# albtad01/NBody-EuroHPC

Measured on AMD Instinct MI355X. Metric: body-interactions/s, higher is better.
Workload: dtype f32; 1 GPU; murb galaxy N=200000 steps=451 dt=3600 soft=2e8 seed=0 fp32 — BASELINE.json configs[2]: N=200000 i=200, 1 x MI355X; n_bodies=200000, parallelism=1 gpu, kernel_variant=8, jsplit=1, sym_waves=4, taper_pct=5, sym_passes=1

## Files before the change

### nbody-eurohpc_amd/csrc/murb_choose.h

```cpp
#ifndef MURB_CHOOSE_H_
#define MURB_CHOOSE_H_

#include <algorithm>
#include <cstddef>

#include "murb_layout.h"
#include "murb_plan.h"

namespace {

struct PlanInputs {
    unsigned long n = 0;
    int world = 1;
    unsigned long slice = 0;
    unsigned long slots = 0;
    int cu_count = 0;
    size_t device_mem = 0;
    int resident_per_cu = 0;
    int variant = 0, jsplit = 0;
    int sym_waves = 0;
    int taper = -1;
    int diag_tri = -1;
    int sym_red = -1;
    int fuse_integrate = 1;
    long sym_pass_mb = 0;
    int tri_div = 0;
};

constexpr int kMaxParts = 64;
constexpr int kNumVariants = 8;
constexpr int kOneSidedVariant = 1;
constexpr int kOneSidedFewBodies = 2;
constexpr int kPersistentVariant = 7;
constexpr int kSymmetricVariant = 8;
constexpr unsigned long kSymmetricMinBodies = 2049;
constexpr int kRowsPerLaunch = kMaxParts / 2;

struct Plan {
    int variant;
    int parts_local, parts_remote;
    bool persistent;
    bool symmetric;
    int split;
    int waves;
    int taper;
    bool diag_tri;
    int red;
    MurbSchedule sched[2];
};

constexpr double kSymFastMaxReach = 0x1p34;
constexpr double kSymFastMinSoft = 0x1p-40;
inline bool sym_wide_needed(double reach, double soft) { return !(reach <= kSymFastMaxReach && soft >= kSymFastMinSoft); }
inline bool sym_wide_chosen(int option, bool needed) { return option < 0 ? needed : option != 0; }

inline int resident_blocks(const PlanInputs& in) { return std::max(in.resident_per_cu, 1) * std::max(in.cu_count, 1); }

inline MurbSchedule make_schedule(const PlanInputs& in, long groups, long tiles, int row_base)
{
    MurbSchedule sc{(int)groups, (int)tiles, 1, row_base};
    const long units = groups * tiles;
    if (units <= 0) { sc.nblocks = 0; return sc; }
    const long slots = resident_blocks(in);
    long rounds = in.jsplit > 0 ? in.jsplit : std::min<long>(8, std::max<long>(1, units / (slots * 8)));
    long nb = std::min(units, slots * rounds);
    nb = std::min(nb, std::max<long>(1, (kRowsPerLaunch - 2) * groups));
    sc.nblocks = (int)std::max<long>(nb, 1);
    return sc;
}

inline int variant_group(int variant)
{
    switch (variant) {
        case kPersistentVariant: return 32;
        case kSymmetricVariant: return 32;
        case 2: case 6: return 16;
        case 5: return 64;
        default: return 32;
    }
}

inline int auto_parts(const PlanInputs& in, int variant, unsigned long i_slots, unsigned long tiles)
{
    if (tiles == 0) return 0;
    const unsigned long groups = (i_slots + variant_group(variant) - 1) / variant_group(variant);
    const unsigned long want_blocks = (unsigned long)std::max(in.cu_count, 1) * 6ul * 24ul;
    unsigned long parts = (want_blocks + groups - 1) / groups;
    parts = std::min(parts, std::max(tiles / 8ul, 1ul));
    parts = std::max(parts, 1ul);
    return (int)std::min<unsigned long>(parts, kMaxParts / 2);
}

inline long sym_items_per_rank(const PlanInputs& in)
{
    const long tb = (long)(in.slice / MURB_SYM_BLOCK), w = in.world;
    return tb * (tb + 1) / 2 + ((w - 1) / 2) * tb * tb + (w > 1 && w % 2 == 0 ? tb * ((tb + 1) / 2) : 0);
}

inline size_t sym_pass_budget(const PlanInputs& in)
{
    if (in.sym_pass_mb > 0) return (size_t)in.sym_pass_mb << 20;
    return in.device_mem ? in.device_mem / 4 : 0;
}

inline size_t sym_row_bytes(const PlanInputs& in, int split)
{
    const size_t tb = in.slice / MURB_SYM_BLOCK, w = (size_t)in.world, far = w / 2;
    size_t rows = tb * tb + (size_t)(split - 1) * tb * (tb - 1) / 2;
    if (w > 1) rows += tb * far * tb + far * tb * (size_t)split * tb;
    return rows * MURB_SYM_BLOCK * 3 * sizeof(float);
}

inline bool fused_one_sided_wins(const PlanInputs& in)
{
    const unsigned long T = in.slots / MURB_SYM_BLOCK;
    return in.fuse_integrate && in.jsplit == 0 && (T <= 4 || T == 6);
}

inline Plan make_plan(const PlanInputs& in)
{
    Plan p{};
    const auto fits = [&](int split) { return in.world == 1 || in.device_mem == 0 || sym_row_bytes(in, split) < in.device_mem / 2; };
    if (in.variant >= 1 && in.variant <= kNumVariants) p.variant = in.variant;
    else if (in.world == 1) p.variant = (in.n >= kSymmetricMinBodies && !fused_one_sided_wins(in) && fits(1)) ? kSymmetricVariant : kOneSidedVariant;
    else p.variant = (sym_items_per_rank(in) >= 400 && fits(1)) ? kSymmetricVariant : (in.slice <= 16384 ? kOneSidedFewBodies : kOneSidedVariant);
    p.symmetric = p.variant == kSymmetricVariant;
    if (p.symmetric) {
        const long items = sym_items_per_rank(in);
        const long want = (in.world > 1 ? 16L : 8L) * 4 * std::max(in.cu_count, 1);
        p.split = (in.jsplit == 1 || in.jsplit == 2 || in.jsplit == 4 || in.jsplit == 8 || in.jsplit == 16)
                      ? in.jsplit
                      : (items >= want ? 1 : (2 * items >= want ? 2 : (in.world == 1 || items >= 1000 ? 4 : (items >= 400 ? 8 : 16))));
        struct SmallPlan { int waves, split, taper; bool diag_tri; };
        static const SmallPlan kSmallPlans[5] = {{8, 4, 30, true}, {4, 4, 5, false}, {4, 8, 5, false}, {8, 8, 30, true}, {4, 16, 5, false}};
        static const signed char kSmallPlanOfBlocks[25] = {4, 4, 4, 3, 3, 3, 4,
                                                           3, 3, 0, 2, 2, 1, 3, 0, 2, 1, 2, 0, 1, 2, 0, 1, 0, 2};
        const int T = (int)(in.slots / MURB_SYM_BLOCK);
        const bool small = in.world == 1 && T <= 27;
        const SmallPlan sp = kSmallPlans[(small && in.cu_count == 256 && T >= 3) ? kSmallPlanOfBlocks[T - 3] : (T < 10 ? 3 : 0)];
        p.waves = (in.sym_waves == 4 || in.sym_waves == 8) ? in.sym_waves : (small ? sp.waves : 4);
        if (in.jsplit == 0 && in.sym_waves == 0 && small) p.split = sp.split;
        while (p.split > 1 && MURB_SYM_BLOCK / p.split < 16 * p.waves) p.split /= 2;
        while (p.split > 1 && !fits(p.split)) p.split /= 2;
        p.taper = in.taper >= 0 ? in.taper : (in.world > 1 ? 0 : (small ? sp.taper : (in.n <= 600000 ? 5 : 0)));
        p.diag_tri = in.diag_tri >= 0 ? in.diag_tri != 0 : (small && sp.diag_tri);
        p.red = in.sym_red >= 0 ? in.sym_red : 1;
        p.persistent = false;
        p.parts_local = p.parts_remote = 0;
        return p;
    }
    const unsigned long tiles_local = in.slice / MURB_TILE_BODIES;
    const unsigned long tiles_remote = (in.slots - in.slice) / MURB_TILE_BODIES;
    p.persistent = p.variant == kPersistentVariant;
    if (p.persistent) {
        unsigned long first, count;
        partition(in.n, in.world, 0, &first, &count);
        const long groups = (long)((count + 31) / 32);
        p.sched[0] = make_schedule(in, groups, (long)tiles_local, 0);
        p.sched[1] = make_schedule(in, groups, (long)tiles_remote, kRowsPerLaunch);
        p.parts_local = p.parts_remote = 0;
        return p;
    }
    if (in.world == 1) {
        p.parts_local = in.jsplit > 0 ? std::min<int>(in.jsplit, (int)std::min<unsigned long>(tiles_local, kMaxParts))
                                      : auto_parts(in, p.variant, in.slice, tiles_local);
        if (in.jsplit == 0 && in.fuse_integrate && p.variant == kOneSidedVariant && in.slots / MURB_SYM_BLOCK <= 6) p.parts_local = 1;
        p.parts_remote = 0;
    } else {
        const unsigned long tiles_all = tiles_local + tiles_remote;
        int total = in.jsplit > 0 ? in.jsplit : auto_parts(in, p.variant, in.slice, tiles_all);
        total = std::max(total, 2);
        int loc = (int)std::max<unsigned long>(1ul, (unsigned long)total * tiles_local / tiles_all);
        int rem = std::max(1, total - loc);
        p.parts_local = (int)std::min<unsigned long>((unsigned long)loc, std::min<unsigned long>(tiles_local, kMaxParts / 2));
        p.parts_remote = (int)std::min<unsigned long>((unsigned long)rem, std::min<unsigned long>(tiles_remote, kMaxParts / 2));
    }
    return p;
}

inline int plan_tri_div(const PlanInputs& in, const Plan& p)
{
    if (in.tri_div > 0) return in.tri_div;
    if (in.world == 1) return 1;
    const long tb = (long)(in.slice / MURB_SYM_BLOCK);
    const long items = tb * (tb + 1) / 2 * p.split / 2;
    const long slots = 4L * std::max(in.cu_count, 1) * 4 / p.waves;
    int div = 1;
    while (div < 4 && items * div < 2 * slots && MURB_SYM_BLOCK / (p.split * div * 2) >= 16 * p.waves) div *= 2;
    return div;
}

inline SymLayoutKey sym_layout_key(const PlanInputs& in, const Plan& p, bool exchange_mode, int overlap, int tri_first_pct, bool xcd_order,
                                   bool pad_aware)
{
    SymLayoutKey k;
    k.split = p.split; k.waves = p.waves; k.taper = p.taper; k.diag_tri = p.diag_tri;
    k.exchange_mode = exchange_mode;
    k.overlap = exchange_mode ? overlap : 0;
    k.tri_first_pct = exchange_mode ? tri_first_pct : 0;
    k.xcd_order = xcd_order;
    k.budget_floats = sym_pass_budget(in) / (3 * sizeof(float));
    k.tri_div = plan_tri_div(in, p);
    k.pad_aware = pad_aware;
    return k;
}

inline int hermite_parts(const PlanInputs& in)
{
    const unsigned long tiles = in.slots / MURB_TILE_BODIES;
    if (in.jsplit > 0) return (int)std::min<unsigned long>((unsigned long)in.jsplit, std::min<unsigned long>(tiles, kMaxParts / 2));
    return auto_parts(in, kOneSidedFewBodies, in.slots, tiles);
}

}

#endif
```

### nbody-eurohpc_amd/csrc/murb_ctx.h

```cpp
#ifndef MURB_CTX_H_
#define MURB_CTX_H_

#include <hip/hip_runtime.h>

#include <vector>

#include "murb_choose.h"
#include "murb_crew.h"
#include "murb_kernels_block.h"
#include "murb_kernels_field.h"
#include "murb_kernels_sym.h"
#include "murb_kernels_tidal.h"
#include "murb_kernels_tracer.h"
#include "murb_kernels_knn.h"
#include "murb_rccl.h"

namespace {

inline int hip_rc(hipError_t e) { return e == hipSuccess ? 0 : -(int)e; }
inline int nccl_rc(int r) { return r == 0 ? 0 : -(3000 + r); }

template <typename... P> inline void release(P*... p) { ((void)hipFree((void*)p), ...); }
inline void release_event(hipEvent_t& e) { if (e) (void)hipEventDestroy(e); e = nullptr; }
inline void release_stream(hipStream_t& s) { if (s) (void)hipStreamDestroy(s); s = nullptr; }
inline void drain(hipStream_t s) { if (s) (void)hipStreamSynchronize(s); }

#define HIP_TRY(expr)                        \
    do {                                     \
        const int rc_ = hip_rc((expr));      \
        if (rc_ != 0) return rc_;            \
    } while (0)
#define RC_TRY(expr)                \
    do {                            \
        const int rc_ = (expr);     \
        if (rc_ != 0) return rc_;   \
    } while (0)

struct SymSet {
    float* part = nullptr;
    size_t comp_stride = 0;
    MurbSymBlockRows* rows = nullptr;
    int nblocks = 0;
    std::vector<SymPass> passes;
};

struct Shard {
    int device = 0;
    int rank = 0;
    unsigned long first = 0, count = 0;
    hipStream_t compute = nullptr, comm = nullptr;
    hipStream_t compute_low = nullptr;
    hipEvent_t ev_integrated = nullptr, ev_gathered = nullptr, ev_tri = nullptr;
    float4* rec[2] = {nullptr, nullptr};
    float4* vel = nullptr;
    float4* accp = nullptr;
    float* acc_out = nullptr;
    float* phi_out = nullptr;
    float* mass = nullptr;
    float* radius = nullptr;
    double* metrics = nullptr;
    double* metrics_host = nullptr;
    MurbSymItem* sym_items = nullptr;
    int sym_items_own = 0, sym_items_total = 0;
    SymLayoutKey key;
    int sym_red = 0;
    int sym_t1 = 0;
    SymSet sym_main;
    SymSet sym_tri;
    float* sym_send = nullptr;
    float* sym_recv = nullptr;
    float* sym_p2p = nullptr;
    float* sym_tri_acc = nullptr;
    double* sym_acc64 = nullptr;
    hipEvent_t ev_rowsum = nullptr, ev_reduced = nullptr;
    rccl_comm_t comm_rccl = nullptr;
    std::vector<hipEvent_t> prof;
    size_t prof_used = 0;
    std::vector<int> prof_kind;
    float4* herm_rec = nullptr;
    float4* herm_vel = nullptr;
    float* herm_a0 = nullptr;
    float* herm_j0 = nullptr;
    float4* herm_part = nullptr;
    int herm_rows = 0;
    MurbEvolveCtl* herm_ctl = nullptr;
    MurbEvolveCtl* herm_ctl_host = nullptr;
    MurbBlockCtl* blk_ctl = nullptr;
    MurbBlockCtl* blk_ctl_host = nullptr;
    unsigned int* blk_ticks = nullptr;
    int* blk_levels = nullptr;
    int* blk_list = nullptr;
    float4* blk_rec = nullptr;
    float4* blk_vel = nullptr;
    float4* blk_part = nullptr;
    size_t blk_rows = 0;
    int* nn_idx = nullptr;
    float* nn_r2 = nullptr;
    MurbEncList* enc = nullptr;
    float* herm_phi = nullptr;
    double* pot_sums = nullptr;
    double* pot_sums_host = nullptr;
    float* fld_in = nullptr;
    float4* fld_pts = nullptr;
    float* fld_out = nullptr;
    size_t fld_points = 0;
    float4* fld_part = nullptr;
    size_t fld_rows = 0;
    float* trc_state = nullptr;
    float4* trc_pts = nullptr;
    size_t trc_cap = 0;
    float4* trc_part = nullptr;
    size_t trc_rows = 0;
    float* knn_part_r2 = nullptr;
    int* knn_part_idx = nullptr;
    size_t knn_part = 0;
    float* knn_list_r2 = nullptr;
    int* knn_list_idx = nullptr;
    size_t knn_list = 0;
    float* knn_rho = nullptr;
    size_t knn_rhos = 0;
    double* knn_sums = nullptr;
    size_t knn_blocks = 0;
    unsigned long sym_launches = 0;
    size_t bytes = 0;
};

template <typename T>
int shard_alloc(Shard& sh, T*& p, size_t bytes, hipStream_t zero_on = nullptr)
{
    if (p) return 0;
    HIP_TRY(hipMalloc((void**)&p, bytes));
    sh.bytes += bytes;
    if (zero_on) HIP_TRY(hipMemsetAsync(p, 0, bytes, zero_on));
    return 0;
}
template <typename T>
void shard_free(Shard& sh, T*& p, size_t bytes)
{
    if (!p) return;
    release(p);
    p = nullptr;
    sh.bytes -= bytes;
}

constexpr int kPeSumBlocks = 256;
constexpr size_t kProfPairs = 4096;

enum ProfKind {
    kProfForce = 0,
    kProfTri1,
    kProfRect,
    kProfTri2,
    kProfReduceScatter,
    kProfAllGather,
    kProfWaitGather,
    kProfWaitReduce,
    kProfStep,
    kProfField,
    kProfTidal,
    kProfTracer,
    kProfKnn,
    kProfKinds
};

}

struct murbhip_ctx {
    PlanInputs in;
    float soft2 = 0.f, g = 0.f;
    int exchange = 0;
    bool rank_mode = false;
    std::vector<Shard> shards;
    ShardCrew* crew = nullptr;
    int cur = 0;
    bool uploaded = false;
    bool gather_pending = false;
    bool reduce_pending = false;
    int profile = 0, overlap = 1;
    int tri_first_pct = 50;
    int xcd_order = 0;
    int evolve_batch = 0;
    int integrator = 0;
    bool herm_current = false;
    bool herm_in_acc_out = false;
    bool herm_proposal = false;
    unsigned long evolve_steps = 0;
    int block_units = 0;
    bool blk_open = false;
    int blk_have_levels = 0;
    float blk_dt_max = 0.f;
    int blk_kmax = 0;
    double blk_steps_per_block = 0;
    double blk_info[4] = {0, 0, 0, 0};
    int nearest = 0;
    float enc_radius = 0.f;
    unsigned long enc_count = 0;
    double enc_time = 0.0;
    int contact = 0;
    int potential = 0;
    long field_chunks = 0;
    long field_batch = 0;
    unsigned long tracers = 0;
    bool trc_current = false;
    long tracer_chunks = 0;
    long tracer_batch = 0;
    int tracer_dt = 0;
    bool lf_half = false;
    bool acc_current = false;
    unsigned long state_serial = 1;
    unsigned long metrics_serial = 0;
    bool metrics_with_phi = false;
    double metrics_sums[MURB_METRIC_VALUES] = {0};
    bool want_pe = false;
    bool pe_current = false;
    float lf_last_dt = 0.f;
    int force_exchange = 0;
    int init_libm_fma = -1;
    int sym_wide = -1;
    bool sym_wide_needed = false;
    int energy_sweep = 0;
    int exchange_p2p = 0;
    int pad_aware = 1;
    int cu_reserve = 0;
    int solo_shard = -1;
    int clock_mhz = 0;
    double interactions_per_launch = 0;
    int async_error = 0;
};

#endif
```

### nbody-eurohpc_amd/csrc/murb_kernels_sym.h

```cpp
#ifndef MURB_KERNELS_SYM_H_
#define MURB_KERNELS_SYM_H_

#include "murb_kernels.h"
#include "murb_sym_types.h"

#ifndef MURB_SYM_STEP_BARRIER
#define MURB_SYM_STEP_BARRIER 1
#endif

struct MurbSymArgs {
    const float4* rec;
    float* part;
    unsigned long comp_stride;
    const MurbSymItem* items;
    int item_first;
    float soft2;
};

__device__ __forceinline__ void murb_swap32(float& a, float& b)
{
    asm volatile("s_nop 1\n\tv_permlane32_swap_b32 %0, %1\n\ts_nop 1" : "+v"(a), "+v"(b));
}
__device__ __forceinline__ void murb_swap16(float& a, float& b)
{
    asm volatile("s_nop 1\n\tv_permlane16_swap_b32 %0, %1\n\ts_nop 1" : "+v"(a), "+v"(b));
}
template <int CTRL> __device__ __forceinline__ float murb_dpp(float v)
{
    return __builtin_bit_cast(float, __builtin_amdgcn_update_dpp(0, __builtin_bit_cast(int, v), CTRL, 0xF, 0xF, true));
}

__device__ __forceinline__ float murb_reduce12(float (&v)[12], int lane)
{
    float w[6];
#pragma unroll
    for (int k = 0; k < 6; ++k) { murb_swap32(v[2 * k], v[2 * k + 1]); w[k] = v[2 * k] + v[2 * k + 1]; }
    float x[3];
#pragma unroll
    for (int m = 0; m < 3; ++m) { murb_swap16(w[2 * m], w[2 * m + 1]); x[m] = w[2 * m] + w[2 * m + 1]; }
    const bool b3 = (lane & 8) != 0, b2 = (lane & 4) != 0;
    const float keep3 = b3 ? x[1] : x[0], send3 = b3 ? x[0] : x[1];
    const float y0 = keep3 + murb_dpp<0x140>(send3);
    const float y1 = x[2] + murb_dpp<0x140>(x[2]);
    const float keep2 = b2 ? y1 : y0, send2 = b2 ? y0 : y1;
    float z = keep2 + murb_dpp<0x141>(send2);
    z += murb_dpp<0x4E>(z);
    z += murb_dpp<0xB1>(z);
    return z;
}

__device__ __forceinline__ float murb_masked(float v, unsigned mask)
{
    float out;
    asm("s_and_b32 %0, %1, %2" : "=s"(out) : "s"(v), "s"(mask) : "scc");
    return out;
}
__device__ __forceinline__ unsigned murb_ones_if_ge(int p, int threshold)
{
    unsigned out;
    asm("s_sub_i32 %0, %1, %2\n\ts_ashr_i32 %0, %0, 31" : "=s"(out) : "s"(threshold), "s"(p + 1) : "scc");
    return out;
}

template <int WIDE = 0>
__device__ __forceinline__ void murb_interact_sym(const murb_f2 xj, const murb_f2 yj, const murb_f2 zj, const murb_f2 gj,
                                                  const float xi, const float yi, const float zi, const float gi,
                                                  const float soft2, murb_f2& aix, murb_f2& aiy, murb_f2& aiz,
                                                  murb_f2& ajx, murb_f2& ajy, murb_f2& ajz)
{
    const murb_f2 dx = xj - xi;
    const murb_f2 dy = yj - yi;
    const murb_f2 dz = zj - zi;
    murb_f2 r2 = __builtin_elementwise_fma(dx, dx, (murb_f2)(soft2));
    r2 = __builtin_elementwise_fma(dy, dy, r2);
    r2 = __builtin_elementwise_fma(dz, dz, r2);
    murb_f2 inv;
    inv.x = __builtin_amdgcn_rsqf(r2.x);
    inv.y = __builtin_amdgcn_rsqf(r2.y);
    murb_f2 fi, fj;
    if constexpr (WIDE) {
        const murb_f2 inv2 = inv * inv;
        fi = (gj * inv) * inv2;
        fj = ((murb_f2)(-gi) * inv) * inv2;
    } else {
        const murb_f2 inv3 = (inv * inv) * inv;
        fi = gj * inv3;
        fj = inv3 * (-gi);
    }
    aix = __builtin_elementwise_fma(fi, dx, aix);
    aiy = __builtin_elementwise_fma(fi, dy, aiy);
    aiz = __builtin_elementwise_fma(fi, dz, aiz);
    ajx = __builtin_elementwise_fma(fj, dx, ajx);
    ajy = __builtin_elementwise_fma(fj, dy, ajy);
    ajz = __builtin_elementwise_fma(fj, dz, ajz);
}

template <int WIDE = 0>
__device__ __forceinline__ void murb_interact_sym_pe(const murb_f2 xj, const murb_f2 yj, const murb_f2 zj, const murb_f2 gj,
                                                     const float xi, const float yi, const float zi, const float gi, const float gi_pe,
                                                     const float soft2, murb_f2& aix, murb_f2& aiy, murb_f2& aiz,
                                                     murb_f2& ajx, murb_f2& ajy, murb_f2& ajz, murb_f2& pe)
{
    const murb_f2 dx = xj - xi;
    const murb_f2 dy = yj - yi;
    const murb_f2 dz = zj - zi;
    murb_f2 r2 = __builtin_elementwise_fma(dx, dx, (murb_f2)(soft2));
    r2 = __builtin_elementwise_fma(dy, dy, r2);
    r2 = __builtin_elementwise_fma(dz, dz, r2);
    murb_f2 inv;
    inv.x = __builtin_amdgcn_rsqf(r2.x);
    inv.y = __builtin_amdgcn_rsqf(r2.y);
    murb_f2 fi, fj, gg;
    if constexpr (WIDE) {
        const murb_f2 inv2 = inv * inv;
        gg = gj * inv;
        fi = gg * inv2;
        fj = ((murb_f2)(-gi) * inv) * inv2;
    } else {
        const murb_f2 inv3 = (inv * inv) * inv;
        fi = gj * inv3;
        fj = inv3 * (-gi);
        gg = gj * inv;
    }
    pe = __builtin_elementwise_fma(gg, (murb_f2)(gi_pe), pe);
    aix = __builtin_elementwise_fma(fi, dx, aix);
    aiy = __builtin_elementwise_fma(fi, dy, aiy);
    aiz = __builtin_elementwise_fma(fi, dz, aiz);
    ajx = __builtin_elementwise_fma(fj, dx, ajx);
    ajy = __builtin_elementwise_fma(fj, dy, ajy);
    ajz = __builtin_elementwise_fma(fj, dz, ajz);
}

__device__ __forceinline__ void murb_interact_sym_phi(const murb_f2 xj, const murb_f2 yj, const murb_f2 zj, const murb_f2 gj,
                                                      const float xi, const float yi, const float zi, const float gi,
                                                      const float soft2, murb_f2& phi_i, murb_f2& phi_j)
{
    const murb_f2 dx = xj - xi;
    const murb_f2 dy = yj - yi;
    const murb_f2 dz = zj - zi;
    murb_f2 r2 = __builtin_elementwise_fma(dx, dx, (murb_f2)(soft2));
    r2 = __builtin_elementwise_fma(dy, dy, r2);
    r2 = __builtin_elementwise_fma(dz, dz, r2);
    murb_f2 inv;
    inv.x = __builtin_amdgcn_rsqf(r2.x);
    inv.y = __builtin_amdgcn_rsqf(r2.y);
    phi_i = __builtin_elementwise_fma(gj, inv, phi_i);
    phi_j = __builtin_elementwise_fma(inv, (murb_f2)(gi), phi_j);
}

template <int WAVES, int ILOAD, int PHI, int RED, int DYN, int WIDE>
__device__ __forceinline__ void murb_sym_walk(const MurbSymArgs& a, const float4* tileA, const float4* tileB, float* stage,
                                              const int lane, const int wave, const int groups_per_wave,
                                              const unsigned int i_block_slot, const unsigned long out_off, const int out_stride,
                                              const float pe_scale, const int p_first,
                                              const int p_sym, murb_f2 (&ajx)[MURB_SYM_STEPS], murb_f2 (&ajy)[MURB_SYM_STEPS],
                                              murb_f2 (&ajz)[MURB_SYM_STEPS])
{
    constexpr int R = MURB_SYM_R;
    constexpr int NV = PHI == 2 ? 13 : 12;
    const float soft2 = a.soft2;
    const int stage_wr = lane;
    const int stage_rd = ((lane >> 2) < NV ? (lane >> 2) : NV - 1) * 80 + (lane & 3) * 4;
    const auto team_sum = [&](int g_of) {
        const float4* src = reinterpret_cast<const float4*>(stage + stage_rd);
        const float4 t0 = src[0], t1 = src[4], t2 = src[8], t3 = src[12];
        murb_f2 s2 = (murb_f2){t0.x, t0.y} + (murb_f2){t0.z, t0.w};
        s2 += (murb_f2){t1.x, t1.y}; s2 += (murb_f2){t1.z, t1.w};
        s2 += (murb_f2){t2.x, t2.y}; s2 += (murb_f2){t2.z, t2.w};
        s2 += (murb_f2){t3.x, t3.y}; s2 += (murb_f2){t3.z, t3.w};
        float z = s2.x + s2.y;
        z += murb_dpp<0xB1>(z);
        z += murb_dpp<0x4E>(z);
        a.part[(unsigned long)out_off + (unsigned long)(g_of * out_stride)] = z;
    };
#pragma unroll 1
    for (int gk = 0; gk < groups_per_wave; ++gk) {
        asm volatile("" ::: "memory");
        const int g = gk * WAVES + wave;
        const unsigned int i_slot = i_block_slot + g * R;
        float xi[R], yi[R], zi[R], gi[R];
#if defined(__HIP_DEVICE_COMPILE__)
        if constexpr (ILOAD == 1) {
            typedef const float4 __attribute__((address_space(4))) * murb_cf4p;
            const murb_cf4p crec = (murb_cf4p)a.rec;
            const unsigned long ra = murb_rec_a((unsigned long)(i_slot >> 1));
#pragma unroll
            for (int h = 0; h < R / 2; ++h) {
                const float4 A = crec[ra + h];
                const float4 B = crec[ra + h + MURB_TILE_PAIRS];
                xi[2 * h] = A.x; xi[2 * h + 1] = A.y;
                yi[2 * h] = A.z; yi[2 * h + 1] = A.w;
                zi[2 * h] = B.x; zi[2 * h + 1] = B.y;
                gi[2 * h] = B.z; gi[2 * h + 1] = B.w;
            }
        } else
#endif
        {
            const unsigned long ra = murb_rec_a((unsigned long)(i_slot >> 1));
#pragma unroll
            for (int h = 0; h < R / 2; ++h) {
                const float4 A = a.rec[ra + h];
                const float4 B = a.rec[ra + h + MURB_TILE_PAIRS];
                xi[2 * h] = A.x; xi[2 * h + 1] = A.y;
                yi[2 * h] = A.z; yi[2 * h + 1] = A.w;
                zi[2 * h] = B.x; zi[2 * h + 1] = B.y;
                gi[2 * h] = B.z; gi[2 * h + 1] = B.w;
            }
#pragma unroll
            for (int r = 0; r < R; ++r) {
                xi[r] = __builtin_bit_cast(float, __builtin_amdgcn_readfirstlane(__builtin_bit_cast(int, xi[r])));
                yi[r] = __builtin_bit_cast(float, __builtin_amdgcn_readfirstlane(__builtin_bit_cast(int, yi[r])));
                zi[r] = __builtin_bit_cast(float, __builtin_amdgcn_readfirstlane(__builtin_bit_cast(int, zi[r])));
                gi[r] = __builtin_bit_cast(float, __builtin_amdgcn_readfirstlane(__builtin_bit_cast(int, gi[r])));
            }
        }
        murb_f2 aix[R], aiy[R], aiz[R];
#pragma unroll
        for (int r = 0; r < R; ++r) { aix[r] = (murb_f2)(0.f); aiy[r] = (murb_f2)(0.f); aiz[r] = (murb_f2)(0.f); }
        murb_f2 pe = (murb_f2)(0.f);

#pragma unroll
        for (int p = 0; p < MURB_SYM_STEPS; ++p) {
            if (DYN == 0 || p >= p_first) {
                const float4 A = tileA[p * 64 + lane];
                const float4 B = tileB[p * 64 + lane];
                const murb_f2 xj = {A.x, A.y}, yj = {A.z, A.w}, zj = {B.x, B.y}, gj = {B.z, B.w};
                const unsigned both = DYN ? murb_ones_if_ge(p, p_sym) : ~0u;
#pragma unroll
                for (int r = 0; r < R; ++r) {
                    const float gie = DYN ? murb_masked(gi[r], both) : gi[r];
                    if constexpr (PHI == 1)
                        murb_interact_sym_phi(xj, yj, zj, gj, xi[r], yi[r], zi[r], gie, soft2, aix[r], ajx[p]);
                    else if constexpr (PHI == 2)
                        murb_interact_sym_pe<WIDE>(xj, yj, zj, gj, xi[r], yi[r], zi[r], gie, gi[r], soft2, aix[r], aiy[r], aiz[r], ajx[p],
                                             ajy[p], ajz[p], pe);
                    else
                        murb_interact_sym<WIDE>(xj, yj, zj, gj, xi[r], yi[r], zi[r], gie, soft2, aix[r], aiy[r], aiz[r], ajx[p], ajy[p],
                                          ajz[p]);
                }
            }
            if (MURB_SYM_STEP_BARRIER) __builtin_amdgcn_sched_barrier(0);
        }

        float v[12];
#pragma unroll
        for (int r = 0; r < R; ++r) {
            v[3 * r + 0] = aix[r].x + aix[r].y;
            v[3 * r + 1] = aiy[r].x + aiy[r].y;
            v[3 * r + 2] = aiz[r].x + aiz[r].y;
        }
        if constexpr (RED == 0) {
            a.part[(unsigned long)out_off + g * R] = murb_reduce12(v, lane);
        } else {
#pragma unroll
            for (int k = 0; k < 12; ++k) stage[k * 80 + stage_wr] = v[k];
            if constexpr (PHI == 2) stage[12 * 80 + stage_wr] = (pe.x + pe.y) * pe_scale;
            team_sum(g);
        }
    }
}

template <int MINW, int WAVES = 4, int ILOAD = 0, int PHI = 0, int RED = 0, int WIDE = 0>
__global__ __launch_bounds__(64 * WAVES, MINW) void murb_force_sym_kernel(const MurbSymArgs a)
{
    constexpr int THREADS = 64 * WAVES;
    __shared__ float4 tileA[MURB_SYM_PAIRS];
    __shared__ float4 tileB[MURB_SYM_PAIRS];
    __shared__ murb_f2 scratch[WAVES / 2][3][MURB_SYM_PAIRS];

    const int lane = threadIdx.x & 63;
    const int wave = __builtin_amdgcn_readfirstlane(threadIdx.x >> 6);

    const MurbSymItem it = a.items[a.item_first + blockIdx.x];
    const int J = __builtin_amdgcn_readfirstlane(it.J);
    const int i_item_slot = __builtin_amdgcn_readfirstlane(it.i_slot0);
    const int groups_per_wave = __builtin_amdgcn_readfirstlane(it.ngroups);
    const int flags = __builtin_amdgcn_readfirstlane(it.flags);
    const bool no_j_side = (flags & 1) != 0;
    const bool triangular = (flags & 2) != 0;
    const int p_first = (flags >> 8) & 15, p_sym = (flags >> 12) & 15;
#ifdef MURB_LAB_BEGIN
    MURB_LAB_BEGIN();
#endif

    {
        const float4* src = a.rec + (unsigned long)J * (MURB_SYM_BLOCK / MURB_TILE_BODIES) * MURB_TILE_F4;
#pragma unroll
        for (int k = threadIdx.x; k < 2 * MURB_TILE_F4; k += THREADS) {
            const int tile = k / MURB_TILE_F4, in = k % MURB_TILE_F4;
            const float4 v = src[k];
            if (in < MURB_TILE_PAIRS) tileA[tile * MURB_TILE_PAIRS + in] = v;
            else tileB[tile * MURB_TILE_PAIRS + in - MURB_TILE_PAIRS] = v;
        }
    }
    __syncthreads();

    murb_f2 ajx[MURB_SYM_STEPS], ajy[MURB_SYM_STEPS], ajz[MURB_SYM_STEPS];
#pragma unroll
    for (int p = 0; p < MURB_SYM_STEPS; ++p) { ajx[p] = (murb_f2)(0.f); ajy[p] = (murb_f2)(0.f); ajz[p] = (murb_f2)(0.f); }

    unsigned long out_off;
    int out_stride = MURB_SYM_R;
    {
        const int b2 = (lane >> 2) & 1, b3 = (lane >> 3) & 1, b4 = (lane >> 4) & 1, b5 = (lane >> 5) & 1;
        int idx = b2 ? 8 + 2 * b4 + b5 : 4 * b3 + 2 * b4 + b5;
        if constexpr (RED != 0) idx = (lane >> 2) < 12 ? (lane >> 2) : 11;
        const int r = idx / 3, c = idx - 3 * r;
        out_off = (unsigned long)c * a.comp_stride + it.ioff + r;
        if constexpr (PHI == 2) {
            static_assert(RED == 1, "the pair potential leaves through the LDS team reduction");
            if ((lane >> 2) >= 12) { out_off = 3ul * a.comp_stride + it.ioff / MURB_SYM_R; out_stride = 1; }
        }
    }
    float* const stage = reinterpret_cast<float*>(&scratch[0][0][0]) + wave * ((PHI == 2 ? 13 : 12) * 80);
    if (triangular)
        murb_sym_walk<WAVES, ILOAD, PHI, RED, 1, WIDE>(a, tileA, tileB, stage, lane, wave, groups_per_wave, (unsigned int)i_item_slot, out_off,
                                                 out_stride, 0.f, p_first, p_sym, ajx, ajy, ajz);
    else
        murb_sym_walk<WAVES, ILOAD, PHI, RED, 0, WIDE>(a, tileA, tileB, stage, lane, wave, groups_per_wave, (unsigned int)i_item_slot, out_off,
                                                 out_stride, (i_item_slot / MURB_SYM_BLOCK == J) ? 0.f : 1.f, 0, 0, ajx, ajy, ajz);

    if (!no_j_side) {
        if constexpr (RED != 0) __syncthreads();
#pragma unroll
        for (int half = WAVES / 2; half >= 1; half >>= 1) {
            if (wave >= half && wave < 2 * half) {
#pragma unroll
                for (int p = 0; p < MURB_SYM_STEPS; ++p) {
                    scratch[wave - half][0][p * 64 + lane] = ajx[p];
                    scratch[wave - half][1][p * 64 + lane] = ajy[p];
                    scratch[wave - half][2][p * 64 + lane] = ajz[p];
                }
            }
            __syncthreads();
            if (wave < half) {
#pragma unroll
                for (int p = 0; p < MURB_SYM_STEPS; ++p) {
                    ajx[p] += scratch[wave][0][p * 64 + lane];
                    ajy[p] += scratch[wave][1][p * 64 + lane];
                    ajz[p] += scratch[wave][2][p * 64 + lane];
                }
            }
            if (half > 1) __syncthreads();
        }
        if (wave == 0) {
            murb_f2* px = reinterpret_cast<murb_f2*>(a.part + it.joff);
            murb_f2* py = reinterpret_cast<murb_f2*>(a.part + a.comp_stride + it.joff);
            murb_f2* pz = reinterpret_cast<murb_f2*>(a.part + 2ul * a.comp_stride + it.joff);
#pragma unroll
            for (int p = 0; p < MURB_SYM_STEPS; ++p) {
                px[p * 64 + lane] = ajx[p];
                if constexpr (PHI != 1) {
                    py[p * 64 + lane] = ajy[p];
                    pz[p * 64 + lane] = ajz[p];
                }
            }
        }
    }
#ifdef MURB_LAB_END
    MURB_LAB_END();
#endif
}

#define MURB_ROWSUM_GROUPS 16
#define MURB_ROWSUM_THREADS (64 * MURB_ROWSUM_GROUPS)
__device__ __forceinline__ bool murb_sym_rowsum_slot(const float* part, unsigned long comp_stride, const MurbSymBlockRows& br,
                                                     unsigned int in_block, int g, int lane,
                                                     double (&red)[MURB_ROWSUM_GROUPS - 1][3][64], double (&total)[3])
{
    double acc[3] = {0.0, 0.0, 0.0};
    for (int idx = g; idx < br.nj; idx += MURB_ROWSUM_GROUPS) {
        const unsigned long o = br.base_j + (unsigned long)idx * MURB_SYM_BLOCK + in_block;
#pragma unroll
        for (int c = 0; c < 3; ++c) acc[c] += (double)part[(unsigned long)c * comp_stride + o];
    }
    for (int idx = g; idx < br.ni; idx += MURB_ROWSUM_GROUPS) {
        const unsigned long o = br.base_i + (unsigned long)idx * MURB_SYM_BLOCK + in_block;
#pragma unroll
        for (int c = 0; c < 3; ++c) acc[c] += (double)part[(unsigned long)c * comp_stride + o];
    }
    if (g > 0) {
#pragma unroll
        for (int c = 0; c < 3; ++c) red[g - 1][c][lane] = acc[c];
    }
    __syncthreads();
    if (g != 0) return false;
#pragma unroll
    for (int c = 0; c < 3; ++c) {
        double t = acc[c];
#pragma unroll
        for (int k = 0; k < MURB_ROWSUM_GROUPS - 1; ++k) t += red[k][c][lane];
        total[c] = t;
    }
    return true;
}

__global__ __launch_bounds__(MURB_ROWSUM_THREADS) void murb_sym_rowsum_kernel(const float* part, unsigned long comp_stride,
                                                                              const MurbSymBlockRows* rows, float* out,
                                                                              unsigned int out_slice_slots)
{
    __shared__ double red[MURB_ROWSUM_GROUPS - 1][3][64];
    const int lane = threadIdx.x & 63, g = threadIdx.x >> 6;
    const unsigned int wg = gridDim.x - 1 - blockIdx.x;
    const MurbSymBlockRows br = rows[wg / (MURB_SYM_BLOCK / 64)];
    const unsigned int in_block = (wg % (MURB_SYM_BLOCK / 64)) * 64 + lane;
    double total[3];
    if (!murb_sym_rowsum_slot(part, comp_stride, br, in_block, g, lane, red, total)) return;
#pragma unroll
    for (int c = 0; c < 3; ++c)
        out[((unsigned long)br.out_slice * 3 + c) * out_slice_slots + (unsigned long)br.out_block * MURB_SYM_BLOCK + in_block] =
            (float)total[c];
}

__global__ __launch_bounds__(MURB_ROWSUM_THREADS) void murb_sym_rowsum_acc_kernel(const float* part, unsigned long comp_stride,
                                                                                  const MurbSymBlockRows* rows, double* acc64,
                                                                                  unsigned int slots)
{
    __shared__ double red[MURB_ROWSUM_GROUPS - 1][3][64];
    const int lane = threadIdx.x & 63, g = threadIdx.x >> 6;
    const unsigned int wg = gridDim.x - 1 - blockIdx.x;
    const MurbSymBlockRows br = rows[wg / (MURB_SYM_BLOCK / 64)];
    const unsigned int in_block = (wg % (MURB_SYM_BLOCK / 64)) * 64 + lane;
    double total[3];
    if (!murb_sym_rowsum_slot(part, comp_stride, br, in_block, g, lane, red, total)) return;
#pragma unroll
    for (int c = 0; c < 3; ++c) acc64[(unsigned long)c * slots + (unsigned long)br.out_block * MURB_SYM_BLOCK + in_block] += total[c];
}

__global__ __launch_bounds__(MURB_ROWSUM_THREADS) void murb_sym_rowsum_integrate_kernel(const float* part, unsigned long comp_stride,
                                                                                        const MurbSymBlockRows* rows,
                                                                                        const MurbIntegrateArgs a)
{
#pragma clang fp contract(off)
    __shared__ double red[MURB_ROWSUM_GROUPS - 1][3][64];
    const int lane = threadIdx.x & 63, g = threadIdx.x >> 6;
    const unsigned int wg = gridDim.x - 1 - blockIdx.x;
    const unsigned int s = wg * 64 + lane;
    const MurbSymBlockRows br = rows[wg / (MURB_SYM_BLOCK / 64)];
    double total[3];
    if (!murb_sym_rowsum_slot(part, comp_stride, br, s % MURB_SYM_BLOCK, g, lane, red, total)) return;
    float ax = (float)total[0], ay = (float)total[1], az = (float)total[2];
    if (a.acc_planes) {
        ax += a.acc_planes[s]; ay += a.acc_planes[a.acc_stride + s]; az += a.acc_planes[2u * a.acc_stride + s];
    }
    a.acc_out[s] = ax;
    a.acc_out[a.acc_stride + s] = ay;
    a.acc_out[2u * a.acc_stride + s] = az;
    if (!a.update_state || (int)s >= a.count) return;

    const unsigned long ra = murb_rec_a((unsigned long)((unsigned int)a.i_first_slot + s) >> 1);
    const unsigned long va = murb_rec_a((unsigned long)(s >> 1));
    const int h = (int)(s & 1u);
    const float4 A = a.rec_in[ra], B = a.rec_in[ra + MURB_TILE_PAIRS];
    const float4 VA = a.vel[va], VB = a.vel[va + MURB_TILE_PAIRS];
    float x = h ? A.y : A.x, y = h ? A.w : A.z, z = h ? B.y : B.x;
    const float gm = h ? B.w : B.z;
    float vx = h ? VA.y : VA.x, vy = h ? VA.w : VA.z, vz = h ? VB.y : VB.x;
    const float dt = a.dt;
    if (a.scheme == 1) {
        const float k = a.kick_dt;
        vx = murb_add_rounded(vx, murb_kick(ax, k)); vy = murb_add_rounded(vy, murb_kick(ay, k)); vz = murb_add_rounded(vz, murb_kick(az, k));
        x = murb_drift(x, vx, 0.f, dt); y = murb_drift(y, vy, 0.f, dt); z = murb_drift(z, vz, 0.f, dt);
    } else {
        const float kx = murb_kick(ax, dt), ky = murb_kick(ay, dt), kz = murb_kick(az, dt);
        x = murb_drift(x, vx, kx, dt); y = murb_drift(y, vy, ky, dt); z = murb_drift(z, vz, kz, dt);
        vx = murb_add_rounded(vx, kx); vy = murb_add_rounded(vy, ky); vz = murb_add_rounded(vz, kz);
    }
    float* oa = reinterpret_cast<float*>(a.rec_out + ra);
    float* ob = reinterpret_cast<float*>(a.rec_out + ra + MURB_TILE_PAIRS);
    oa[h] = x; oa[2 + h] = y; ob[h] = z; ob[2 + h] = gm;
    float* wa = reinterpret_cast<float*>(a.vel + va);
    float* wb = reinterpret_cast<float*>(a.vel + va + MURB_TILE_PAIRS);
    wa[h] = vx; wa[2 + h] = vy; wb[h] = vz;
}

#define MURB_PE_DIAG_SPLIT 16
__global__ __launch_bounds__(256) void murb_sym_pe_diag_kernel(const float4* rec, int first_block, float soft2, double* out)
{
    __shared__ float4 body[MURB_SYM_BLOCK];
    __shared__ double red[4];
    const int t = threadIdx.x, block = first_block + blockIdx.x / MURB_PE_DIAG_SPLIT, y = blockIdx.x % MURB_PE_DIAG_SPLIT;
    for (int k = t; k < MURB_SYM_BLOCK; k += 256) {
        const unsigned long slot = (unsigned long)block * MURB_SYM_BLOCK + k;
        const unsigned long ra = murb_rec_a(slot >> 1);
        const float4 A = rec[ra], B = rec[ra + MURB_TILE_PAIRS];
        body[k] = (k & 1) ? make_float4(A.y, A.w, B.y, B.w) : make_float4(A.x, A.z, B.x, B.z);
    }
    __syncthreads();
    const int i = 64 * y + (t & 63), wave = t >> 6;
    const float4 me = body[i];
    double acc = 0.0;
#pragma unroll 4
    for (int off = 128 * wave + 1; off <= 128 * wave + 128; ++off) {
        const float4 o = body[(i + off) & (MURB_SYM_BLOCK - 1)];
        const float dx = o.x - me.x, dy = o.y - me.y, dz = o.z - me.z;
        const float inv = __builtin_amdgcn_rsqf(fmaf(dz, dz, fmaf(dy, dy, fmaf(dx, dx, soft2))));
        const float term = o.w * inv;
        acc += (double)(off == MURB_SYM_BLOCK / 2 ? 0.5f * term : term);
    }
    acc *= (double)me.w;
#pragma unroll
    for (int off = 32; off >= 1; off >>= 1) acc += __shfl_down(acc, off, 64);
    if ((t & 63) == 0) red[wave] = acc;
    __syncthreads();
    if (t == 0) out[blockIdx.x] = ((red[0] + red[1]) + red[2]) + red[3];
}

// ... 40 lines not shown
```

### nbody-eurohpc_amd/csrc/murb_plan.h

```cpp
#ifndef MURB_PLAN_H_
#define MURB_PLAN_H_

#include <cstddef>
#include <map>
#include <utility>
#include <vector>

#include "murb_schedule.h"
#include "murb_sym_types.h"

namespace {

struct SymPass {
    int item_first = 0, item_count = 0;
    int table_first = 0, table_count = 0;
    size_t floats = 0;
};

inline std::vector<std::pair<size_t, size_t>> cut_passes(const std::vector<SymPiece>& pieces, size_t budget_floats)
{
    std::vector<std::pair<size_t, size_t>> out;
    size_t first = 0, used = 0, k = 0;
    while (k < pieces.size()) {
        size_t e = k, rows = 0;
        int last_block = -1;
        while (e < pieces.size() && pieces[e].J == pieces[k].J) {
            rows += pieces[e].j_side() ? 1 : 0;
            if (pieces[e].i_slot0 / MURB_SYM_BLOCK != last_block) { ++rows; last_block = pieces[e].i_slot0 / MURB_SYM_BLOCK; }
            ++e;
        }
        const size_t need = rows * MURB_SYM_BLOCK;
        if (budget_floats && used > 0 && used + need > budget_floats) { out.emplace_back(first, k); first = k; used = 0; }
        used += need;
        k = e;
    }
    out.emplace_back(first, pieces.size());
    return out;
}

template <class OutOf>
size_t layout_sym_set(const std::vector<SymPiece>& pieces, size_t first, size_t end, int waves, std::vector<MurbSymItem>& items,
                      std::vector<MurbSymBlockRows>& table, OutOf out_of)
{
    std::map<int, int> index;
    for (size_t k = first; k < end; ++k) { index[pieces[k].i_slot0 / MURB_SYM_BLOCK] = 0; if (pieces[k].j_side()) index[pieces[k].J] = 0; }
    table.assign(index.size(), MurbSymBlockRows{});
    { int e = 0; for (auto& kv : index) { kv.second = e; const auto o = out_of(kv.first); table[e].out_slice = o.first; table[e].out_block = o.second; ++e; } }
    std::vector<std::map<int, int>> irow(index.size());
    std::vector<int> item_irow(end - first), item_jrow(end - first);
    for (size_t k = first; k < end; ++k) {
        const SymPiece& pc = pieces[k];
        const int bi = index[pc.i_slot0 / MURB_SYM_BLOCK];
        auto f = irow[bi].find(pc.J);
        if (f == irow[bi].end()) f = irow[bi].emplace(pc.J, table[bi].ni++).first;
        item_irow[k - first] = f->second;
        item_jrow[k - first] = pc.j_side() ? table[index[pc.J]].nj++ : -1;
    }
    size_t floats = 0;
    for (MurbSymBlockRows& br : table) {
        br.base_j = floats; floats += (size_t)br.nj * MURB_SYM_BLOCK;
        br.base_i = floats; floats += (size_t)br.ni * MURB_SYM_BLOCK;
    }
    for (size_t k = first; k < end; ++k) {
        const SymPiece& pc = pieces[k];
        MurbSymItem& it = items[k];
        it.i_slot0 = pc.i_slot0;
        it.ngroups = pc.len / (waves * MURB_SYM_R);
        it.J = pc.J;
        it.flags = pc.flags;
        const MurbSymBlockRows& bi = table[index[pc.i_slot0 / MURB_SYM_BLOCK]];
        it.ioff = bi.base_i + (size_t)item_irow[k - first] * MURB_SYM_BLOCK + (size_t)(pc.i_slot0 % MURB_SYM_BLOCK);
        it.joff = pc.j_side() ? table[index[pc.J]].base_j + (size_t)item_jrow[k - first] * MURB_SYM_BLOCK : 0;
    }
    return floats;
}

struct SymHostLayout {
    std::vector<MurbSymItem> items;
    int own = 0, t1 = 0;
    std::vector<MurbSymBlockRows> table_main, table_tri;
    size_t floats_main = 0, floats_tri = 0;
    std::vector<SymPass> passes;
};

struct SymLayoutKey {
    int split = 1, waves = 4, taper = 0;
    bool diag_tri = false;
    bool exchange_mode = false;
    int overlap = 0, tri_first_pct = 0;
    bool xcd_order = false;
    size_t budget_floats = 0;
    int tri_div = 1;
    bool pad_aware = true;
    bool operator==(const SymLayoutKey& o) const
    {
        return split == o.split && waves == o.waves && taper == o.taper && diag_tri == o.diag_tri && exchange_mode == o.exchange_mode &&
               overlap == o.overlap && tri_first_pct == o.tri_first_pct && xcd_order == o.xcd_order && budget_floats == o.budget_floats &&
               tri_div == o.tri_div && pad_aware == o.pad_aware;
    }
};

inline void plan_sym_layout(int W, int r, const SymFill& fill, const SymLayoutKey& key, SymHostLayout& L)
{
    const int tb = fill.tb;
    std::vector<int> flat;
    int own = 0;
    size_t t1 = 0;
    std::vector<SymPiece> pieces;
    std::vector<size_t> piece_ends;
    const auto build_pieces = [&](bool interleaved) {
        sym_schedule_items(W, r, tb, key.split, fill, flat, &own, interleaved);
        const size_t n_all = flat.size() / 2;
        t1 = (key.exchange_mode && key.overlap == 1) ? (size_t)((long)own * key.tri_first_pct / 100) : 0;
        std::vector<size_t> launch_ends;
        std::vector<int> launch_div;
        if (key.exchange_mode) {
            if (t1 > 0) { launch_ends.push_back(t1); launch_div.push_back(key.tri_div); }
            if ((size_t)own > t1) { launch_ends.push_back((size_t)own); launch_div.push_back(key.tri_div); }
            if (n_all > (size_t)own) { launch_ends.push_back(n_all); launch_div.push_back(1); }
        } else {
            launch_ends.push_back(n_all);
        }
        sym_pieces(flat, key.split, key.taper, 16 * key.waves, key.diag_tri, fill, launch_ends, pieces, piece_ends, launch_div);
    };
    build_pieces(key.xcd_order);
    if (!key.exchange_mode && key.xcd_order && cut_passes(pieces, key.budget_floats).size() > 1) build_pieces(false);
    size_t own_pieces = pieces.size();
    if (key.exchange_mode && flat.size() / 2 > (size_t)own) own_pieces = piece_ends.size() >= 2 ? piece_ends[piece_ends.size() - 2] : 0;
    L.items.assign(pieces.size(), MurbSymItem{});
    L.table_main.clear(); L.table_tri.clear();
    L.floats_main = L.floats_tri = 0;
    if (key.exchange_mode) {
        L.floats_tri = layout_sym_set(pieces, 0, own_pieces, key.waves, L.items, L.table_tri, [&](int b) { return std::make_pair(0, b - r * tb); });
        L.floats_main = layout_sym_set(pieces, own_pieces, pieces.size(), key.waves, L.items, L.table_main,
                                       [&](int b) { return std::make_pair(b / tb, b % tb); });
        L.passes.assign(1, SymPass{(int)own_pieces, (int)(pieces.size() - own_pieces), 0, (int)L.table_main.size(), L.floats_main});
    } else {
        L.passes.clear();
        std::vector<MurbSymBlockRows> table;
        for (const auto& range : cut_passes(pieces, key.budget_floats)) {
            const size_t floats = layout_sym_set(pieces, range.first, range.second, key.waves, L.items, table, [&](int b) { return std::make_pair(0, b); });
            L.passes.push_back(SymPass{(int)range.first, (int)(range.second - range.first), (int)L.table_main.size(), (int)table.size(), floats});
            L.table_main.insert(L.table_main.end(), table.begin(), table.end());
            L.floats_main = std::max(L.floats_main, floats);
        }
    }
    L.own = (int)own_pieces;
    L.t1 = t1 > 0 ? (int)piece_ends[0] : 0;
}

}

#endif
```

### nbody-eurohpc_amd/csrc/murb_schedule.h

```cpp
#ifndef MURB_SCHEDULE_H_
#define MURB_SCHEDULE_H_

#include <algorithm>
#include <vector>

#include "murb_layout.h"

namespace {

inline void partition(unsigned long n, int world, int rank, unsigned long* first, unsigned long* count)
{
    const unsigned long base = n / (unsigned long)world, rem = n % (unsigned long)world;
    const unsigned long r = (unsigned long)rank;
    *count = base + (r < rem ? 1 : 0);
    *first = r * base + std::min(r, rem);
}

inline unsigned long slice_slots(unsigned long n, int world)
{
    unsigned long first, count;
    partition(n, world, 0, &first, &count);
    return murb_round_up_tile(std::max(count, 1ul));
}

constexpr int kXcds = 8;
inline void xcd_interleave(std::vector<int>& flat, size_t first_item, size_t end_item)
{
    const size_t n = end_item - first_item;
    if (n < 2 * kXcds) return;
    std::vector<int> src(flat.begin() + 2 * first_item, flat.begin() + 2 * end_item);
    auto start = [&](size_t x) { return x * n / kXcds; };
    size_t p = 0;
    for (size_t k = 0; p < n; ++k)
        for (size_t x = 0; x < (size_t)kXcds && p < n; ++x) {
            if (start(x) + k >= start(x + 1)) continue;
            const size_t it = start(x) + k;
            flat[2 * (first_item + p)] = src[2 * it];
            flat[2 * (first_item + p) + 1] = src[2 * it + 1];
            ++p;
        }
}

struct SymFill {
    int tb = 0;
    std::vector<int> count;
    int of(int block) const
    {
        const int left = count[(size_t)(block / tb)] - (block % tb) * MURB_SLICE_ALIGN;
        return left <= 1 ? 1 : (left >= MURB_SLICE_ALIGN ? MURB_SLICE_ALIGN : left);
    }
};
inline SymFill sym_fill(unsigned long n, int world, bool aware = true)
{
    SymFill f;
    f.tb = (int)(slice_slots(n, world) / MURB_SLICE_ALIGN);
    for (int s = 0; s < world; ++s) {
        unsigned long first, count;
        partition(n, world, s, &first, &count);
        f.count.push_back(aware ? (int)count : f.tb * MURB_SLICE_ALIGN);
    }
    return f;
}

inline void sym_orient(const SymFill& fill, int def_i, int def_j, int* i_block, int* j_block)
{
    const bool swap = def_i != def_j && fill.of(def_j) < fill.of(def_i);
    *i_block = swap ? def_j : def_i;
    *j_block = swap ? def_i : def_j;
}
inline void sym_push_block_pair(const SymFill& fill, int split, int i_block, int j_block, std::vector<int>& flat)
{
    const int len = MURB_SLICE_ALIGN / split, real = fill.of(i_block);
    for (int q = 0; q < split && q * len < real; ++q) { flat.push_back(i_block * split + q); flat.push_back(j_block); }
}

inline void sym_schedule_items(int world, int rank, int tb, int split, const SymFill& fill, std::vector<int>& flat, int* own, bool xcd_order = false)
{
    const int W = world, r = rank;
    flat.clear();
    for (int j = 0; j < tb; ++j)
        for (int a = 0; a <= j; ++a) {
            int ib, jb;
            sym_orient(fill, r * tb + a, r * tb + j, &ib, &jb);
            sym_push_block_pair(fill, split, ib, jb, flat);
        }
    *own = (int)flat.size() / 2;
    for (int d = 1; d <= W / 2; ++d) {
        const int s = (r + d) % W;
        if (s == r) continue;
        const bool shared = (W % 2 == 0) && d == W / 2;
        const int lo = std::min(r, s);
        int hb = (tb + 1) / 2;
        if (shared) {
            long total = 0, acc = 0, best = -1;
            for (int a = 0; a < tb; ++a) total += fill.of(lo * tb + a);
            for (int h = 0; h <= tb; ++h) {
                const long off = 2 * acc > total ? 2 * acc - total : total - 2 * acc;
                if (best < 0 || off <= best) { best = off; hb = h; }
                if (h < tb) acc += fill.of(lo * tb + h);
            }
        }
        std::vector<int> swapped;
        for (int a = 0; a < tb; ++a) {
            const size_t row_first = flat.size();
            for (int j = 0; j < tb; ++j) {
                if (shared && !((r == lo) ? (a < hb) : (j >= hb))) continue;
                int ib, jb;
                sym_orient(fill, r * tb + a, s * tb + j, &ib, &jb);
                if (ib == r * tb + a) { flat.push_back(ib); flat.push_back(jb); }
                else sym_push_block_pair(fill, split, ib, jb, swapped);
            }
            const std::vector<int> row(flat.begin() + (long)row_first, flat.end());
            flat.resize(row_first);
            const int len = MURB_SLICE_ALIGN / split, real = fill.of(r * tb + a);
            for (int q = 0; q < split && q * len < real; ++q)
                for (size_t k = 0; k < row.size(); k += 2) { flat.push_back(row[k] * split + q); flat.push_back(row[k + 1]); }
        }
        flat.insert(flat.end(), swapped.begin(), swapped.end());
    }
    if (!xcd_order) return;
    const size_t n_own = (size_t)*own, n_all = flat.size() / 2;
    if (W == 1) { xcd_interleave(flat, 0, n_all); return; }
    xcd_interleave(flat, 0, n_own / 2);
    xcd_interleave(flat, n_own / 2, n_own);
    xcd_interleave(flat, n_own, n_all);
}

struct SymPiece {
    int i_slot0, len, J, flags;
    bool diag() const { return i_slot0 / MURB_SLICE_ALIGN == J; }
    bool j_side() const { return (flags & 1) == 0; }
};
constexpr int kSymStepBodies = 128;

inline void sym_pieces(const std::vector<int>& flat, int split, int taper_pct, int min_len, bool diag_tri, const SymFill& fill,
                       const std::vector<size_t>& launch_ends, std::vector<SymPiece>& out, std::vector<size_t>& piece_launch_ends,
                       const std::vector<int>& launch_div = std::vector<int>())
{
    const int len = MURB_SLICE_ALIGN / split;
    out.clear();
    piece_launch_ends.clear();
    size_t first = 0;
    for (size_t l = 0; l < launch_ends.size(); ++l) {
        const size_t end = launch_ends[l];
        const int base_div = l < launch_div.size() ? launch_div[l] : 1;
        const double total = (double)(end - first);
        for (size_t k = first; k < end; ++k) {
            const int isub = flat[2 * k], J = flat[2 * k + 1];
            const bool diag = isub / split == J;
            const double before = (double)(k - first) / (total > 0 ? total : 1.0);
            int div = 1;
            while (div < base_div && len / (2 * div) >= min_len) div *= 2;
            if (taper_pct > 0) {
                const double left = 1.0 - before;
                for (double f = taper_pct / 100.0; left <= f && len / (2 * div) >= min_len; f *= 0.5) div *= 2;
            }
            if (diag && diag_tri)
                while (len / div > kSymStepBodies && len / (2 * div) >= min_len) div *= 2;
            const int real_end = (isub / split) * MURB_SLICE_ALIGN + fill.of(isub / split);
            for (int q = 0; q < div; ++q) {
                SymPiece pc{isub * len + q * (len / div), len / div, J, diag ? 1 : 0};
                if (pc.i_slot0 >= real_end) break;
                if (pc.i_slot0 + pc.len > real_end) pc.len = (real_end - pc.i_slot0 + min_len - 1) / min_len * min_len;
                if (diag && diag_tri && pc.len <= kSymStepBodies) {
                    const int in_block = pc.i_slot0 % MURB_SLICE_ALIGN;
                    const int a = in_block / kSymStepBodies, b = (in_block + pc.len + kSymStepBodies - 1) / kSymStepBodies;
                    pc.flags = 2 | (a << 8) | (b << 12) | (b >= MURB_SLICE_ALIGN / kSymStepBodies ? 1 : 0);
                }
                out.push_back(pc);
            }
        }
        piece_launch_ends.push_back(out.size());
        first = end;
    }
}

}

#endif
```

### nbody-eurohpc_amd/csrc/murb_sym_types.h

```cpp
#ifndef MURB_SYM_TYPES_H_
#define MURB_SYM_TYPES_H_

#define MURB_SYM_BLOCK 1024
#define MURB_SYM_PAIRS (MURB_SYM_BLOCK / 2)
#define MURB_SYM_STEPS (MURB_SYM_PAIRS / 64)
#define MURB_SYM_R 4

struct MurbSymItem {
    int i_slot0;
    int ngroups;
    int J;
    int flags;
    unsigned long ioff;
    unsigned long joff;
};


#define MURB_SYM_MAX_RANKS 64
struct MurbSymBlockRows {
    unsigned long base_i, base_j;
    int ni, nj;
    int out_slice, out_block;
};

#endif
```

### nbody-eurohpc_amd/csrc/murbhip.hip

```cpp
#include <hip/hip_runtime.h>

#include <algorithm>
#include <cmath>
#include <cstdio>
#include <cstdlib>
#include <cstring>
#include <functional>
#include <new>
#include <string>
#include <type_traits>
#include <vector>

#include "../../include/murbhip.h"
#include "../../include/murbfield.h"
#include "../../include/murbtidal.h"
#include "../../include/murbknn.h"
#include "../../include/murbtracer.h"
#include "murb_init.h"
#include "murb_ctx.h"

namespace {

constexpr int kPotentialKernel = 100;

inline bool is_idle(const murbhip_ctx* c, const Shard& sh) { return c->solo_shard >= 0 && sh.rank != c->solo_shard; }

template <int MODE, int R, int WAVES, int STAGE>
int launch_force_t(const MurbForceArgs& a, int i_slots, hipStream_t s)
{
    const dim3 grid((unsigned)((i_slots + WAVES * R - 1) / (WAVES * R)), (unsigned)a.nchunks, 1);
    hipLaunchKernelGGL((murb_force_kernel<MODE, R, WAVES, STAGE>), grid, dim3(WAVES * 64), 0, s, a);
    return hip_rc(hipGetLastError());
}

int launch_force(int variant, const MurbForceArgs& a, int i_slots, hipStream_t s)
{
    switch (variant) {
        case 1: return launch_force_t<MURB_MODE_PK_LDS, 8, 4, 4>(a, i_slots, s);
        case 2: return launch_force_t<MURB_MODE_PK_LDS, 4, 4, 4>(a, i_slots, s);
        case 3: return launch_force_t<MURB_MODE_PK_DIRECT, 8, 4, 1>(a, i_slots, s);
        case 4: return launch_force_t<MURB_MODE_SC_LDS, 8, 4, 4>(a, i_slots, s);
        case 5: return launch_force_t<MURB_MODE_PK_LDS, 16, 4, 4>(a, i_slots, s);
        case 6: return launch_force_t<MURB_MODE_PK_DIRECT, 4, 4, 1>(a, i_slots, s);
        case kPotentialKernel:
            return i_slots <= 8192 ? launch_force_t<MURB_MODE_PHI, 2, 8, 4>(a, i_slots, s) : launch_force_t<MURB_MODE_PHI, 8, 4, 4>(a, i_slots, s);
        default: return MURBHIP_E_INVALID;
    }
}
template <int R, int WAVES = 4>
int launch_force_integrate_t(const MurbForceArgs& a, const MurbIntegrateArgs& ia, int i_slots, hipStream_t s)
{
    const dim3 grid((unsigned)((i_slots + WAVES * R - 1) / (WAVES * R)), 1, 1);
    hipLaunchKernelGGL((murb_force_integrate_kernel<R, WAVES, 4>), grid, dim3(64 * WAVES), 0, s, a, ia);
    return hip_rc(hipGetLastError());
}
int launch_force_integrate(const MurbForceArgs& a, const MurbIntegrateArgs& ia, int i_slots, hipStream_t s)
{
    if (i_slots <= 4096) return launch_force_integrate_t<2, 8>(a, ia, i_slots, s);
    if (i_slots <= 6144) return launch_force_integrate_t<2>(a, ia, i_slots, s);
    if (i_slots <= 8192) return launch_force_integrate_t<4>(a, ia, i_slots, s);
    return launch_force_integrate_t<8>(a, ia, i_slots, s);
}
int launch_persistent(const MurbForceArgs& a, const MurbSchedule& sc, hipStream_t s)
{
    hipLaunchKernelGGL((murb_force_persistent<8, 4, 4>), dim3((unsigned)sc.nblocks), dim3(256), 0, s, a, sc);
    return hip_rc(hipGetLastError());
}

Plan current_plan(murbhip_ctx* c)
{
    if (c->in.variant == kPersistentVariant && c->in.resident_per_cu == 0) {
        int n = 0;
        if (hipOccupancyMaxActiveBlocksPerMultiprocessor(&n, murb_force_persistent<8, 4, 4>, 256, 0) != hipSuccess || n < 1)
            n = 4;
        c->in.resident_per_cu = n;
    }
    return make_plan(c->in);
}

int crew_run(murbhip_ctx* c, const std::function<int(Shard&)>& job)
{
    return c->crew->run([&](int i) -> int {
        Shard& sh = c->shards[(size_t)i];
        if (c->crew->threads() == 0) RC_TRY(hip_rc(hipSetDevice(sh.device)));
        return job(sh);
    });
}

int span_begin(murbhip_ctx* c, Shard& sh, int kind, hipStream_t stream, int* rc)
{
    const int level = (kind <= kProfTri2) ? 1 : 2;
    if (c->profile < level || sh.prof_used + 2 > sh.prof.size()) return -1;
    const int k = (int)(sh.prof_used / 2);
    sh.prof_used += 2;
    sh.prof_kind[(size_t)k] = kind;
    const int r = hip_rc(hipEventRecord(sh.prof[(size_t)2 * k], stream));
    if (r && !*rc) *rc = r;
    return k;
}
int span_end(Shard& sh, int span, hipStream_t stream)
{
    if (span < 0) return 0;
    return hip_rc(hipEventRecord(sh.prof[(size_t)2 * span + 1], stream));
}
int timed_wait(murbhip_ctx* c, Shard& sh, int kind, hipStream_t stream, hipEvent_t ev)
{
    int rc = 0;
    const int sp = span_begin(c, sh, kind, stream, &rc);
    RC_TRY(rc);
    HIP_TRY(hipStreamWaitEvent(stream, ev, 0));
    return span_end(sh, sp, stream);
}

int build_sym_schedule(murbhip_ctx* c, Shard& sh, const Plan& p);
int ensure_accp(murbhip_ctx* c, Shard& sh) { return shard_alloc(sh, sh.accp, (size_t)kMaxParts * c->in.slice * sizeof(float4), sh.compute); }
struct MetricsLayout {
    size_t blocks, pe_main, pe_tri, pe_diag, own_blocks, total;
};
MetricsLayout metrics_layout(const murbhip_ctx* c)
{
    MetricsLayout l{};
    l.blocks = (c->in.slice + 255) / 256;
    l.pe_main = l.blocks * MURB_METRIC_VALUES;
    l.pe_tri = l.pe_main + kPeSumBlocks;
    l.pe_diag = l.pe_tri + kPeSumBlocks;
    l.own_blocks = c->in.slice / MURB_SYM_BLOCK;
    l.total = l.pe_diag + l.own_blocks * MURB_PE_DIAG_SPLIT;
    return l;
}

int enqueue_sym_passes(murbhip_ctx* c, Shard& sh, bool potential);
int enqueue_sym_launch(murbhip_ctx* c, Shard& sh, int first, int count, bool own_triangle_rows = false,
                       hipStream_t stream = nullptr, bool potential = false, size_t comp_stride = 0, int kind = kProfForce);

inline void note_interactions(murbhip_ctx* c, const Shard& sh, double v) { if (&sh == &c->shards[0]) c->interactions_per_launch = v; }

int enqueue_force(murbhip_ctx* c, Shard& sh, const Plan& p, int which, const MurbIntegrateArgs* then = nullptr, bool* fused = nullptr)
{
    MurbForceArgs a{};
    if (!p.symmetric) RC_TRY(ensure_accp(c, sh));
    a.rec = sh.rec[c->cur];
    a.accp = sh.accp;
    a.i_first_slot = (int)((unsigned long)sh.rank * c->in.slice);
    a.acc_stride = (unsigned int)c->in.slice;
    a.soft2 = c->soft2;
    const int tiles_local = (int)(c->in.slice / MURB_TILE_BODIES);
    const int tiles_all = (int)(c->in.slots / MURB_TILE_BODIES);
    if (which == 0) {
        a.tiles = MurbTileRange{sh.rank * tiles_local, tiles_local, tiles_local, 0};
        a.chunk_first = 0;
        a.nchunks = p.parts_local;
    } else {
        a.tiles = MurbTileRange{0, tiles_all - tiles_local, sh.rank * tiles_local, tiles_local};
        a.chunk_first = p.parts_local;
        a.nchunks = p.parts_remote;
    }
    const int i_slots = (int)sh.count;
    if (p.symmetric) {
        if (which != 0) return 0;
        RC_TRY(build_sym_schedule(c, sh, p));
        if (sh.sym_main.passes.size() > 1) {
            RC_TRY(enqueue_sym_passes(c, sh, false));
            note_interactions(c, sh, (double)c->in.n * (double)c->in.n / (double)sh.sym_main.passes.size());
            return 0;
        }
        RC_TRY(enqueue_sym_launch(c, sh, 0, sh.sym_items_total));
        note_interactions(c, sh, (double)c->in.n * (double)c->in.n);
        return 0;
    }
    if (p.persistent) {
        const MurbSchedule& sc = p.sched[which];
        if (sc.nblocks <= 0 || a.tiles.count <= 0) return 0;
        int rc = 0;
        const int sp = span_begin(c, sh, kProfForce, sh.compute, &rc);
        RC_TRY(rc);
        RC_TRY(launch_persistent(a, sc, sh.compute));
        RC_TRY(span_end(sh, sp, sh.compute));
    } else {
        if (a.nchunks <= 0 || a.tiles.count <= 0) return 0;
        int rc = 0;
        const int sp = span_begin(c, sh, kProfForce, sh.compute, &rc);
        RC_TRY(rc);
        if (then && fused && p.variant == kOneSidedVariant && a.nchunks == 1 && then->nparts == 1) {
            RC_TRY(launch_force_integrate(a, *then, i_slots, sh.compute));
            *fused = true;
        } else {
            RC_TRY(launch_force(p.variant, a, i_slots, sh.compute));
        }
        RC_TRY(span_end(sh, sp, sh.compute));
    }
    note_interactions(c, sh, (double)i_slots * (double)a.tiles.count * MURB_TILE_BODIES);
    return 0;
}

inline float leapfrog_kick(const murbhip_ctx* c, float dt) { return c->lf_half ? 0.5f * (c->lf_last_dt + dt) : 0.5f * dt; }

MurbIntegrateArgs integrate_args(const murbhip_ctx* c, const Shard& sh, int nparts, float dt, int update_state, int scheme = -1,
                                 float* acc_out = nullptr)
{
    MurbIntegrateArgs a{};
    a.scheme = scheme >= 0 ? scheme : c->integrator;
    a.kick_dt = leapfrog_kick(c, dt);
    a.rec_in = sh.rec[c->cur];
    a.rec_out = sh.rec[c->cur ^ 1];
    a.vel = sh.vel;
    a.accp = sh.accp;
    a.acc_out = acc_out ? acc_out : sh.acc_out;
    a.i_first_slot = (int)((unsigned long)sh.rank * c->in.slice);
    a.count = (int)sh.count;
    a.nparts = nparts;
    a.acc_stride = (unsigned int)c->in.slice;
    a.dt = dt;
    a.update_state = update_state;
    return a;
}

int enqueue_integrate(murbhip_ctx* c, Shard& sh, int nparts, float dt, int update_state, const Plan* plan = nullptr,
                      int scheme = -1, float* acc_out = nullptr, bool acc_from_out = false)
{
    MurbIntegrateArgs a = integrate_args(c, sh, nparts, dt, update_state, scheme, acc_out);
    if (plan && plan->persistent) {
        a.group_bodies = 32;
        a.sched[0] = plan->sched[0];
        a.nsched = 1;
        if (c->in.world > 1 && plan->sched[1].nblocks > 0) { a.sched[1] = plan->sched[1]; a.nsched = 2; }
    }
    if (acc_from_out) a.acc_planes = sh.acc_out;
    if (plan && plan->symmetric && sh.sym_main.passes.size() > 1) {
        a.acc64 = sh.sym_acc64;
        a.acc64_stride = (unsigned int)c->in.slots;
    } else if (plan && plan->symmetric) {
        hipLaunchKernelGGL(murb_sym_rowsum_integrate_kernel, dim3((unsigned)(c->in.slots / 64)), dim3(MURB_ROWSUM_THREADS), 0, sh.compute,
                           sh.sym_main.part, sh.sym_main.comp_stride, sh.sym_main.rows, a);
        return hip_rc(hipGetLastError());
    }
    if (!acc_from_out && !a.acc64) { RC_TRY(ensure_accp(c, sh)); a.accp = sh.accp; }
    const unsigned pairs = (unsigned)(c->in.slice / 2);
    hipLaunchKernelGGL(murb_integrate_kernel, dim3((pairs + 255) / 256), dim3(256), 0, sh.compute, a);
    return hip_rc(hipGetLastError());
}

int shard_exchange(murbhip_ctx* c, Shard& sh, int buf, int failed)
{
    const size_t slice_f4 = c->in.slice;
    const size_t slice_bytes = slice_f4 * sizeof(float4);
    const bool idle = is_idle(c, sh);
    int rc = failed;
    if (!rc && !idle) rc = hip_rc(hipEventRecord(sh.ev_integrated, sh.compute));
    if (c->exchange == 0) c->crew->meet();
    if (rc) return rc;
    int span = -1;
    if (c->exchange == 1) {
        HIP_TRY(hipStreamWaitEvent(sh.comm, sh.ev_integrated, 0));
        span = span_begin(c, sh, kProfAllGather, sh.comm, &rc);
        RC_TRY(rc);
        float4* base = sh.rec[buf];
        if (c->exchange_p2p && c->in.world > 1) {
            Rccl& r = rccl();
            RC_TRY(nccl_rc(r.GroupStart()));
            for (int d = 1; d < c->in.world; ++d) {
                const int to = (sh.rank + d) % c->in.world, from = (sh.rank - d + c->in.world) % c->in.world;
                RC_TRY(nccl_rc(r.Send(base + (size_t)sh.rank * slice_f4, slice_f4 * 4, kRcclFloat, to, sh.comm_rccl, sh.comm)));
                RC_TRY(nccl_rc(r.Recv(base + (size_t)from * slice_f4, slice_f4 * 4, kRcclFloat, from, sh.comm_rccl, sh.comm)));
            }
            RC_TRY(nccl_rc(r.GroupEnd()));
        } else {
            RC_TRY(nccl_rc(rccl().AllGather(base + (size_t)sh.rank * slice_f4, base, slice_f4 * 4, kRcclFloat, sh.comm_rccl, sh.comm)));
        }
    } else {
        if (idle) return 0;
        for (Shard& peer : c->shards) {
            if (&peer == &sh || is_idle(c, peer)) continue;
            HIP_TRY(hipStreamWaitEvent(sh.comm, peer.ev_integrated, 0));
        }
        HIP_TRY(hipStreamWaitEvent(sh.comm, sh.ev_integrated, 0));
        span = span_begin(c, sh, kProfAllGather, sh.comm, &rc);
        RC_TRY(rc);
        for (Shard& peer : c->shards) {
            if (&peer == &sh) continue;
            const size_t off = (size_t)peer.rank * slice_f4;
            if (peer.device == sh.device)
                HIP_TRY(hipMemcpyAsync(sh.rec[buf] + off, peer.rec[buf] + off, slice_bytes, hipMemcpyDeviceToDevice, sh.comm));
            else
                HIP_TRY(hipMemcpyPeerAsync(sh.rec[buf] + off, sh.device, peer.rec[buf] + off, peer.device, slice_bytes, sh.comm));
        }
    }
    RC_TRY(span_end(sh, span, sh.comm));
    if (!idle) HIP_TRY(hipEventRecord(sh.ev_gathered, sh.comm));
    return 0;
}

inline size_t sym_part_bytes(size_t floats) { return (3 * floats + floats / MURB_SYM_R + 1) * sizeof(float); }

void free_sym_set(Shard& sh, SymSet& st)
{
    shard_free(sh, st.part, sym_part_bytes(st.comp_stride));
    shard_free(sh, st.rows, (size_t)st.nblocks * sizeof(MurbSymBlockRows));
    st = SymSet{};
}

int upload_sym_set(Shard& sh, SymSet& st, const std::vector<MurbSymBlockRows>& table, size_t floats)
{
    st.comp_stride = floats;
    st.nblocks = (int)table.size();
    if (floats == 0) return 0;
    RC_TRY(shard_alloc(sh, st.part, sym_part_bytes(floats), sh.compute));
    RC_TRY(shard_alloc(sh, st.rows, table.size() * sizeof(MurbSymBlockRows)));
    HIP_TRY(hipMemcpy(st.rows, table.data(), table.size() * sizeof(MurbSymBlockRows), hipMemcpyHostToDevice));
    return 0;
}

inline bool exchange_mode(const murbhip_ctx* c) { return c->in.world > 1 || c->force_exchange; }
SymLayoutKey layout_key(const murbhip_ctx* c, const Plan& p)
{
    return sym_layout_key(c->in, p, exchange_mode(c), c->overlap, c->tri_first_pct, c->xcd_order != 0, c->pad_aware != 0);
}

inline bool sym_schedule_stale(const Shard& sh, const SymLayoutKey& key) { return !sh.sym_items || !(sh.key == key); }
int drain_for_rebuild(murbhip_ctx* c, const Plan& p)
{
    if (!p.symmetric) return 0;
    const SymLayoutKey key = layout_key(c, p);
    for (const Shard& sh : c->shards)
        if (sh.sym_items && sym_schedule_stale(sh, key)) return murbhip_sync(c);
    return 0;
}

int build_sym_schedule(murbhip_ctx* c, Shard& sh, const Plan& p)
{
    const SymLayoutKey key = layout_key(c, p);
    sh.sym_red = p.red;
    if (!sym_schedule_stale(sh, key)) return 0;
    shard_free(sh, sh.sym_items, (size_t)sh.sym_items_total * sizeof(MurbSymItem));
    free_sym_set(sh, sh.sym_main);
    free_sym_set(sh, sh.sym_tri);

    SymHostLayout L;
    plan_sym_layout(c->in.world, sh.rank, sym_fill(c->in.n, c->in.world, key.pad_aware), key, L);
    if (!key.exchange_mode && L.passes.size() == 1 && (int)L.table_main.size() != (int)(c->in.slots / MURB_SYM_BLOCK))
        return MURBHIP_E_STATE;
    RC_TRY(upload_sym_set(sh, sh.sym_tri, L.table_tri, L.floats_tri));
    RC_TRY(upload_sym_set(sh, sh.sym_main, L.table_main, L.floats_main));
    sh.sym_main.passes = L.passes;
    if (L.passes.size() > 1) RC_TRY(shard_alloc(sh, sh.sym_acc64, 3 * c->in.slots * sizeof(double)));
    sh.sym_items_own = L.own;
    sh.sym_items_total = (int)L.items.size();
    sh.sym_t1 = L.t1;
    RC_TRY(shard_alloc(sh, sh.sym_items, L.items.size() * sizeof(MurbSymItem)));
    HIP_TRY(hipMemcpy(sh.sym_items, L.items.data(), L.items.size() * sizeof(MurbSymItem), hipMemcpyHostToDevice));
    sh.key = key;
    if (key.exchange_mode) {
        const int W = c->in.world;
        const size_t chunk = (size_t)3 * c->in.slice * sizeof(float);
        RC_TRY(shard_alloc(sh, sh.sym_send, chunk * W));
        RC_TRY(shard_alloc(sh, sh.sym_recv, chunk));
        RC_TRY(shard_alloc(sh, sh.sym_tri_acc, chunk));
        if (W > 1) RC_TRY(shard_alloc(sh, sh.sym_p2p, chunk * (size_t)(W / 2), sh.compute));
        if (!sh.ev_rowsum) HIP_TRY(hipEventCreateWithFlags(&sh.ev_rowsum, hipEventDisableTiming));
        if (!sh.ev_reduced) HIP_TRY(hipEventCreateWithFlags(&sh.ev_reduced, hipEventDisableTiming));
        HIP_TRY(hipMemsetAsync(sh.sym_send, 0, chunk * W, sh.compute));
    }
    return 0;
}

template <int WAVES, int WIDE>
void launch_sym_t(int form, int count, hipStream_t stream, const MurbSymArgs& sa)
{
    const dim3 grid((unsigned)count), block(64 * WAVES);
    if (form == 1) hipLaunchKernelGGL((murb_force_sym_kernel<4, WAVES, 1, 1>), grid, block, 0, stream, sa);
    else if (form == 2) hipLaunchKernelGGL((murb_force_sym_kernel<4, WAVES, 1, 2, 1, WIDE>), grid, block, 0, stream, sa);
    else if (form == 3) hipLaunchKernelGGL((murb_force_sym_kernel<4, WAVES, 1, 0, 1, WIDE>), grid, block, 0, stream, sa);
    else hipLaunchKernelGGL((murb_force_sym_kernel<4, WAVES, 1, 0, 0, WIDE>), grid, block, 0, stream, sa);
}

int enqueue_sym_launch(murbhip_ctx* c, Shard& sh, int first, int count, bool own_triangle_rows, hipStream_t stream,
                       bool potential, size_t comp_stride, int kind)
{
    if (count <= 0) return 0;
    if (!stream) stream = sh.compute;
    ++sh.sym_launches;
    const SymSet& st = own_triangle_rows ? sh.sym_tri : sh.sym_main;
    MurbSymArgs sa{};
    sa.rec = sh.rec[c->cur];
    sa.part = st.part;
    sa.comp_stride = comp_stride ? comp_stride : st.comp_stride;
    sa.items = sh.sym_items;
    sa.item_first = first;
    sa.soft2 = c->soft2;
    const bool with_pe = !potential && c->want_pe;
    const bool timed = stream == sh.compute && !potential;
    int rc_span = 0;
    const int sp = timed ? span_begin(c, sh, kind, stream, &rc_span) : -1;
    RC_TRY(rc_span);
    const int form = potential ? 1 : (with_pe ? 2 : (sh.sym_red == 1 ? 3 : 0));
    const bool wide = sym_wide_chosen(c->sym_wide, c->sym_wide_needed);
    if (sh.key.waves == 8) { if (wide) launch_sym_t<8, 1>(form, count, stream, sa); else launch_sym_t<8, 0>(form, count, stream, sa); }
    else { if (wide) launch_sym_t<4, 1>(form, count, stream, sa); else launch_sym_t<4, 0>(form, count, stream, sa); }
    RC_TRY(hip_rc(hipGetLastError()));
    RC_TRY(span_end(sh, sp, stream));
    return 0;
}

int enqueue_sym_rowsum(const SymSet& st, float* out, unsigned int out_slice_slots, hipStream_t stream)
{
    if (st.nblocks <= 0) return 0;
    hipLaunchKernelGGL(murb_sym_rowsum_kernel, dim3((unsigned)st.nblocks * (MURB_SYM_BLOCK / 64)), dim3(MURB_ROWSUM_THREADS), 0, stream,
                       st.part, st.comp_stride, st.rows, out, out_slice_slots);
    return hip_rc(hipGetLastError());
}

int shard_reduce_scatter(murbhip_ctx* c, Shard& sh)
{
    const unsigned int chunk_floats = (unsigned int)(3 * c->in.slice);
    const bool idle = is_idle(c, sh);
    int rc = 0, span = -1;
    if (c->exchange == 1 && c->exchange_p2p && c->in.world > 1) {
        Rccl& r = rccl();
        const int W = c->in.world, D = W / 2;
        HIP_TRY(hipStreamWaitEvent(sh.comm, sh.ev_rowsum, 0));
        span = span_begin(c, sh, kProfReduceScatter, sh.comm, &rc);
        RC_TRY(rc);
        RC_TRY(nccl_rc(r.GroupStart()));
        for (int d = 1; d <= D; ++d) {
            const int to = (sh.rank + d) % W, from = (sh.rank - d + W) % W;
            RC_TRY(nccl_rc(r.Send(sh.sym_send + (size_t)to * chunk_floats, chunk_floats, kRcclFloat, to, sh.comm_rccl, sh.comm)));
            RC_TRY(nccl_rc(r.Recv(sh.sym_p2p + (size_t)(d - 1) * chunk_floats, chunk_floats, kRcclFloat, from, sh.comm_rccl, sh.comm)));
        }
        RC_TRY(nccl_rc(r.GroupEnd()));
        hipLaunchKernelGGL(murb_sym_chunk_sum_kernel, dim3((chunk_floats + 255) / 256), dim3(256), 0, sh.comm,
                           sh.sym_send + (size_t)sh.rank * chunk_floats, sh.sym_p2p, D, chunk_floats, sh.sym_recv);
        RC_TRY(hip_rc(hipGetLastError()));
    } else if (c->exchange == 1) {
        HIP_TRY(hipStreamWaitEvent(sh.comm, sh.ev_rowsum, 0));
        span = span_begin(c, sh, kProfReduceScatter, sh.comm, &rc);
        RC_TRY(rc);
        RC_TRY(nccl_rc(rccl().ReduceScatter(sh.sym_send, sh.sym_recv, chunk_floats, kRcclFloat, kRcclSum, sh.comm_rccl, sh.comm)));
    } else {
        if (idle) return 0;
        const int W = c->in.world, D = W / 2;
        MurbPeerPtrs peers{};
        peers.n = 0;
        for (int d = 0; d <= D; ++d) {
            const int from = (sh.rank - d + W) % W;
            if (d > 0 && from == sh.rank) break;
            for (Shard& peer : c->shards)
                if (peer.rank == from) { peers.p[peers.n++] = peer.sym_send; HIP_TRY(hipStreamWaitEvent(sh.comm, peer.ev_rowsum, 0)); }
        }
        span = span_begin(c, sh, kProfReduceScatter, sh.comm, &rc);
        RC_TRY(rc);
        hipLaunchKernelGGL(murb_sym_peer_sum_kernel, dim3((chunk_floats + 255) / 256), dim3(256), 0, sh.comm, peers,
                           (unsigned long)sh.rank * chunk_floats, chunk_floats, sh.sym_recv);
        RC_TRY(hip_rc(hipGetLastError()));
    }
    RC_TRY(span_end(sh, span, sh.comm));
    if (!idle) HIP_TRY(hipEventRecord(sh.ev_reduced, sh.comm));
    return 0;
}

int wait_send_buffer_free(murbhip_ctx* c, Shard& sh)
{
    if (!c->reduce_pending) return 0;
    if (c->exchange == 0) {
        const int W = c->in.world, D = W / 2;
        for (Shard& peer : c->shards)
            if ((peer.rank - sh.rank + W) % W <= D) HIP_TRY(hipStreamWaitEvent(sh.compute, peer.ev_reduced, 0));
    } else HIP_TRY(hipStreamWaitEvent(sh.compute, sh.ev_reduced, 0));
    return 0;
}

int shard_iteration_sym_multi(murbhip_ctx* c, Shard& sh, const Plan& p, float dt, int update_state)
{
    const bool idle = is_idle(c, sh);
    const bool copies = c->exchange == 0;
    int rc = build_sym_schedule(c, sh, p);
    const int own = sh.sym_items_own, t1 = sh.sym_t1;
    int step_span = -1;
    if (!rc && !idle) rc = [&]() -> int {
        int r = 0;
        step_span = span_begin(c, sh, kProfStep, sh.compute, &r);
        RC_TRY(r);
        if (c->overlap == 2) {
            if (c->gather_pending || c->reduce_pending) HIP_TRY(hipStreamWaitEvent(sh.compute_low, sh.ev_integrated, 0));
            RC_TRY(enqueue_sym_launch(c, sh, 0, own, true, sh.compute_low));
            RC_TRY(enqueue_sym_rowsum(sh.sym_tri, sh.sym_tri_acc, (unsigned int)c->in.slice, sh.compute_low));
            HIP_TRY(hipEventRecord(sh.ev_tri, sh.compute_low));
        }
        RC_TRY(enqueue_sym_launch(c, sh, 0, t1, true, nullptr, false, 0, kProfTri1));
        if (c->gather_pending) RC_TRY(timed_wait(c, sh, kProfWaitGather, sh.compute, sh.ev_gathered));
        RC_TRY(enqueue_sym_launch(c, sh, own, sh.sym_items_total - own, false, nullptr, false, 0, kProfRect));
        RC_TRY(wait_send_buffer_free(c, sh));
        RC_TRY(enqueue_sym_rowsum(sh.sym_main, sh.sym_send, (unsigned int)c->in.slice, sh.compute));
        HIP_TRY(hipEventRecord(sh.ev_rowsum, sh.compute));
        const int launches = (t1 > 0) + (own - t1 > 0 || c->overlap == 2) + (sh.sym_items_total - own > 0);
        note_interactions(c, sh, (double)sh.count * (double)c->in.n / (double)std::max(launches, 1));
        return 0;
    }();
    if (copies) c->crew->meet();
    if (!rc) rc = shard_reduce_scatter(c, sh);
    if (!rc && !idle) rc = [&]() -> int {
        if (c->overlap == 2) {
            HIP_TRY(hipStreamWaitEvent(sh.compute, sh.ev_tri, 0));
        } else {
            RC_TRY(enqueue_sym_launch(c, sh, t1, own - t1, true, nullptr, false, 0, kProfTri2));
        }
        RC_TRY(timed_wait(c, sh, kProfWaitReduce, sh.compute, sh.ev_reduced));
        MurbIntegrateArgs a = integrate_args(c, sh, 0, dt, update_state);
        a.acc_planes = sh.sym_recv;
        if (c->overlap == 2) {
            a.acc_planes2 = sh.sym_tri_acc;
            hipLaunchKernelGGL(murb_integrate_kernel, dim3((unsigned)((c->in.slice / 2 + 255) / 256)), dim3(256), 0, sh.compute, a);
        } else {
            hipLaunchKernelGGL(murb_sym_rowsum_integrate_kernel, dim3((unsigned)(c->in.slice / 64)), dim3(MURB_ROWSUM_THREADS), 0, sh.compute,
                               sh.sym_tri.part, sh.sym_tri.comp_stride, sh.sym_tri.rows, a);
        }
        RC_TRY(hip_rc(hipGetLastError()));
        RC_TRY(span_end(sh, step_span, sh.compute));
        if (!update_state) HIP_TRY(hipEventRecord(sh.ev_integrated, sh.compute));
        return 0;
    }();
    if (update_state) rc = shard_exchange(c, sh, c->cur ^ 1, rc);
    return rc;
}

int enqueue_sym_passes(murbhip_ctx* c, Shard& sh, bool potential)
{
    HIP_TRY(hipMemsetAsync(sh.sym_acc64, 0, 3 * c->in.slots * sizeof(double), sh.compute));
    const bool with_pe = !potential && c->want_pe && sh.metrics;
    bool first = true;
    for (const SymPass& ps : sh.sym_main.passes) {
        float* const pe_plane = sh.sym_main.part + 3 * ps.floats;
        const size_t pe_count = ps.floats / MURB_SYM_R + 1;
        if (with_pe) HIP_TRY(hipMemsetAsync(pe_plane, 0, pe_count * sizeof(float), sh.compute));
        RC_TRY(enqueue_sym_launch(c, sh, ps.item_first, ps.item_count, false, nullptr, potential, ps.floats));
        if (with_pe) {
            hipLaunchKernelGGL(murb_sym_pe_sum_kernel, dim3(kPeSumBlocks), dim3(1024), 0, sh.compute, pe_plane, (unsigned long)pe_count,
                               sh.metrics + metrics_layout(c).pe_main, first ? 0 : 1);
            RC_TRY(hip_rc(hipGetLastError()));
            first = false;
        }
        hipLaunchKernelGGL(murb_sym_rowsum_acc_kernel, dim3((unsigned)ps.table_count * (MURB_SYM_BLOCK / 64)), dim3(MURB_ROWSUM_THREADS), 0,
                           sh.compute, sh.sym_main.part, ps.floats, sh.sym_main.rows + ps.table_first, sh.sym_acc64, (unsigned int)c->in.slots);
        RC_TRY(hip_rc(hipGetLastError()));
    }
    return 0;
}

int shard_potential_sym_multi(murbhip_ctx* c, Shard& sh, const Plan& p)
// ... 845 lines not shown
        hipLaunchKernelGGL(murb_field_pack_kernel, dim3((unsigned)((padded + 255) / 256)), dim3(256), 0, sh.compute, pa);
        MurbKnnArgs ka{};
        ka.rec = sh.rec[c->cur];
        ka.pts = sh.fld_pts;
        ka.part_r2 = sh.knn_part_r2;
        ka.part_idx = sh.knn_part_idx;
        ka.groups = (int)(padded / MURB_FIELD_GROUP);
        const long grid_full = block_grid(c) / 5 * 4;
        ka.chunks = (int)std::min<long>(l.chunks, std::max<long>(1, (grid_full + ka.groups - 1) / ka.groups));
        ka.tiles = l.tiles;
        ka.count = (int)c->in.n;
        ka.k = k;
        ka.stride = (unsigned int)padded;
        ka.soft2 = c->soft2;
        const long units = (long)ka.groups * ka.chunks;
        const unsigned grid = (unsigned)std::max(1l, std::min<long>(units, grid_full));
        int rc = 0;
        const int sp = span_begin(c, sh, kProfKnn, sh.compute, &rc);
        RC_TRY(rc);
        hipLaunchKernelGGL((murb_knn_sweep_kernel<kHermiteR, kHermiteWaves, kKnnStage>), dim3(grid), dim3(kHermiteWaves * 64), 0,
                           sh.compute, ka);
        RC_TRY(span_end(sh, sp, sh.compute));
        const dim3 per_point((unsigned)((bn + 255) / 256));
        hipLaunchKernelGGL(murb_knn_rows_kernel, per_point, dim3(256), 0, sh.compute, (const float*)ka.part_r2,
                           (const int*)ka.part_idx, sh.knn_list_idx, sh.knn_list_r2, (int)bn, ka.chunks, ka.stride, k);
        float* const rho = want_rho ? sh.knn_rho + (rho_all ? first : 0ul) : nullptr;
        if (rho)
            hipLaunchKernelGGL(murb_knn_density_kernel, per_point, dim3(256), 0, sh.compute, (const int*)sh.knn_list_idx,
                               (const float*)sh.knn_list_r2, (const float*)sh.mass, rho, (int)bn, k, c->soft2);
        RC_TRY(hip_rc(hipGetLastError()));
        HIP_TRY(hipStreamSynchronize(sh.compute));
        if (out_idx) HIP_TRY(hipMemcpy(out_idx + first * k, sh.knn_list_idx, bn * k * sizeof(int), hipMemcpyDeviceToHost));
        if (out_r2) HIP_TRY(hipMemcpy(out_r2 + first * k, sh.knn_list_r2, bn * k * sizeof(float), hipMemcpyDeviceToHost));
        if (out_rho) HIP_TRY(hipMemcpy(out_rho + first, rho, bn * sizeof(float), hipMemcpyDeviceToHost));
    }
    return 0;
}

int knn_centre(murbhip_ctx* c, int k, double* out8)
{
    const float* const none[3] = {nullptr, nullptr, nullptr};
    const unsigned long n = c->in.n;
    RC_TRY(knn_run(c, k, n, none, nullptr, true, nullptr, nullptr, nullptr, true));
    Shard& sh = c->shards[0];
    const size_t blocks = (n + 255) / 256;
    RC_TRY(grow(sh, sh.knn_sums, sh.knn_blocks, blocks * MURB_KNN_CENTRE_VALUES));
    std::vector<double> rows(blocks * MURB_KNN_CENTRE_VALUES);
    double sum[MURB_KNN_CENTRE_VALUES], x[3] = {0.0, 0.0, 0.0};
    for (int pass = 0; pass < 2; ++pass) {
        hipLaunchKernelGGL(murb_knn_centre_kernel, dim3((unsigned)blocks), dim3(256), 0, sh.compute, (const float4*)sh.rec[c->cur],
                           (const float*)sh.knn_rho, sh.knn_sums, (int)n, pass, x[0], x[1], x[2]);
        RC_TRY(hip_rc(hipGetLastError()));
        HIP_TRY(hipMemcpyAsync(rows.data(), sh.knn_sums, rows.size() * sizeof(double), hipMemcpyDeviceToHost, sh.compute));
        HIP_TRY(hipStreamSynchronize(sh.compute));
        double s[MURB_KNN_CENTRE_VALUES] = {0};
        for (size_t b = 0; b < blocks; ++b)
            for (int e = 0; e < MURB_KNN_CENTRE_VALUES; ++e) s[e] += rows[b * MURB_KNN_CENTRE_VALUES + e];
        if (pass == 0) {
            for (int e = 0; e < MURB_KNN_CENTRE_VALUES; ++e) sum[e] = s[e];
            for (int e = 0; e < 3; ++e) x[e] = sum[2 + e] / sum[0];
            out8[5] = sum[0];
            out8[6] = sum[5];
            out8[7] = (double)n - sum[5];
            if (sum[0] == 0.0) {
                for (int e = 0; e < 5; ++e) out8[e] = std::numeric_limits<double>::quiet_NaN();
                return 0;
            }
        } else {
            for (int e = 0; e < 3; ++e) out8[e] = x[e];
            out8[3] = std::sqrt(s[0] / sum[1]);
            out8[4] = sum[1] / sum[0];
        }
    }
    return 0;
}

inline bool all_or_none(std::initializer_list<const void*> group)
{
    size_t set = 0;
    for (const void* q : group) set += q != nullptr;
    return set == 0 || set == group.size();
}

inline int field_state(const murbhip_ctx* c)
{
    return !c->uploaded || c->in.world != 1 || c->shards.size() != 1 || c->blk_open ? MURBHIP_E_STATE : 0;
}

}

extern "C" {

int murbhip_version(void) { return 103; }

const char* murbhip_error_string(int code)
{
    static thread_local char buf[160];
    if (code == 0) return "success";
    if (code == MURBHIP_E_INVALID) return "murbhip: invalid argument";
    if (code == MURBHIP_E_STATE) return "murbhip: call made in the wrong state (upload first?)";
    if (code == MURBHIP_E_NO_DEVICE) return "murbhip: no usable HIP device";
    if (code == MURBHIP_E_NO_RCCL) return "murbhip: librccl could not be loaded";
    if (code == MURBHIP_E_NOMEM) return "murbhip: host allocation failed";
    if (code <= -3000 && code > -4000) {
        Rccl& r = rccl();
        snprintf(buf, sizeof buf, "RCCL error %d: %s", -code - 3000,
                 (r.ok && r.GetErrorString) ? r.GetErrorString(-code - 3000) : "?");
        return buf;
    }
    if (code < 0 && code > -2000) {
        snprintf(buf, sizeof buf, "HIP error %d: %s", -code, hipGetErrorString((hipError_t)(-code)));
        return buf;
    }
    snprintf(buf, sizeof buf, "murbhip: unknown code %d", code);
    return buf;
}

int murbhip_partition(unsigned long n, int world, int rank, unsigned long* first, unsigned long* count)
{
    if (world < 1 || rank < 0 || rank >= world || !first || !count) return MURBHIP_E_INVALID;
    partition(n, world, rank, first, count);
    return 0;
}

unsigned long murbhip_slice_slots(unsigned long n, int world) { return world < 1 ? 0 : slice_slots(n, world); }

unsigned long murbhip_slot_of_body(unsigned long n, int world, unsigned long i)
{
    if (world < 1 || i >= n) return ~0ul;
    const unsigned long base = n / (unsigned long)world, rem = n % (unsigned long)world;
    unsigned long r, first;
    if (i < rem * (base + 1)) { r = i / (base + 1); first = r * (base + 1); }
    else { r = rem + (base ? (i - rem * (base + 1)) / base : 0); first = rem * (base + 1) + (r - rem) * base; }
    return r * slice_slots(n, world) + (i - first);
}

int murbhip_schedule_items(unsigned long n, int world, int rank, int split, int* pairs, unsigned long capacity,
                           unsigned long* count, unsigned long* own_count)
{
    if (world < 1 || world > MURB_SYM_MAX_RANKS || rank < 0 || rank >= world || !count || !own_count) return MURBHIP_E_INVALID;
    if (split != 1 && split != 2 && split != 4 && split != 8 && split != 16) return MURBHIP_E_INVALID;
    std::vector<int> flat;
    int own = 0;
    sym_schedule_items(world, rank, (int)(slice_slots(n, world) / MURB_SYM_BLOCK), split, sym_fill(n, world), flat, &own);
    *count = flat.size() / 2;
    *own_count = (unsigned long)own;
    if (pairs) {
        if (capacity < flat.size() / 2) return MURBHIP_E_INVALID;
        std::memcpy(pairs, flat.data(), flat.size() * sizeof(int));
    }
    return 0;
}

int murbhip_schedule_layout(unsigned long n, int world, int rank, int split, int waves, int taper_pct, int tri_first_pct,
                            int exchange_mode, long* items, unsigned long item_capacity, unsigned long* item_count, long* rows,
                            unsigned long row_capacity, unsigned long* row_count, unsigned long* floats_main,
                            unsigned long* floats_tri)
{
    if (world < 1 || world > MURB_SYM_MAX_RANKS || rank < 0 || rank >= world || !item_count || !row_count) return MURBHIP_E_INVALID;
    if (split != 1 && split != 2 && split != 4 && split != 8 && split != 16) return MURBHIP_E_INVALID;
    if ((waves != 4 && waves != 8) || taper_pct < 0 || (taper_pct & 0xff) > 100 || taper_pct > 0x7ff || tri_first_pct < 0 || tri_first_pct > 100)
        return MURBHIP_E_INVALID;
    if (MURB_SYM_BLOCK / split < 16 * waves) return MURBHIP_E_INVALID;
    SymHostLayout L;
    SymLayoutKey key;
    key.split = split; key.waves = waves; key.taper = taper_pct & 0xff; key.diag_tri = (taper_pct & 0x100) != 0;
    key.exchange_mode = exchange_mode != 0 || world > 1;
    key.overlap = 1; key.tri_first_pct = tri_first_pct; key.tri_div = 1 << ((taper_pct >> 9) & 3);
    plan_sym_layout(world, rank, sym_fill(n, world), key, L);
    *item_count = L.items.size();
    *row_count = L.table_main.size() + L.table_tri.size();
    if (floats_main) *floats_main = L.floats_main;
    if (floats_tri) *floats_tri = L.floats_tri;
    if (items) {
        if (item_capacity < L.items.size()) return MURBHIP_E_INVALID;
        const bool ex = key.exchange_mode;
        for (size_t k = 0; k < L.items.size(); ++k) {
            const MurbSymItem& it = L.items[k];
            long* o = items + 8 * k;
            o[0] = it.i_slot0; o[1] = (long)it.ngroups * waves * MURB_SYM_R; o[2] = it.J; o[3] = it.flags;
            o[4] = (ex && (int)k < L.own) ? 1 : 0;
            o[5] = (long)it.ioff; o[6] = (long)it.joff;
            o[7] = !ex ? 0 : ((int)k < L.t1 ? 0 : ((int)k < L.own ? 1 : 2));
        }
    }
    if (rows) {
        if (row_capacity < *row_count) return MURBHIP_E_INVALID;
        size_t e = 0;
        for (int set = 0; set < 2; ++set)
            for (const MurbSymBlockRows& br : (set == 0 ? L.table_main : L.table_tri)) {
                long* o = rows + 7 * e++;
                o[0] = set; o[1] = br.out_slice; o[2] = br.out_block; o[3] = (long)br.base_i; o[4] = br.ni; o[5] = (long)br.base_j; o[6] = br.nj;
            }
    }
    return 0;
}

int murbhip_device_count(int* count)
{
    if (!count) return MURBHIP_E_INVALID;
    *count = 0;
    return hip_rc(hipGetDeviceCount(count));
}

int murbhip_create(murbhip_ctx** out, unsigned long n, float soft, float g, int device)
{
    const int rank0 = 0;
    return create_common(out, n, soft, g, 1, 1, &device, &rank0, 0, false);
}

int murbhip_create_sharded(murbhip_ctx** out, unsigned long n, float soft, float g, int ndev, const int* devices,
                           int exchange)
{
    if (ndev < 1 || ndev > 64 || !devices || (exchange != 0 && exchange != 1)) return MURBHIP_E_INVALID;
    if ((unsigned long)ndev > n) return MURBHIP_E_INVALID;
    std::vector<int> ranks(ndev);
    for (int i = 0; i < ndev; ++i) ranks[i] = i;
    if (exchange == 1) {
        if (!rccl().ok) return MURBHIP_E_NO_RCCL;
    }
    RC_TRY(create_common(out, n, soft, g, ndev, ndev, devices, ranks.data(), exchange, false));
    if (exchange == 1 && ndev > 1) {
        std::vector<rccl_comm_t> comms(ndev);
        const int rc = nccl_rc(rccl().CommInitAll(comms.data(), ndev, devices));
        if (rc != 0) { murbhip_destroy(*out); *out = nullptr; return rc; }
        for (int i = 0; i < ndev; ++i) (*out)->shards[i].comm_rccl = comms[i];
    }
    return 0;
}

int murbhip_unique_id(void* id_out)
{
    if (!id_out) return MURBHIP_E_INVALID;
    Rccl& r = rccl();
    if (!r.ok) return MURBHIP_E_NO_RCCL;
    rccl_id_t id;
    RC_TRY(nccl_rc(r.GetUniqueId(&id)));
    std::memcpy(id_out, &id, sizeof id);
    return 0;
}

int murbhip_create_rank(murbhip_ctx** out, unsigned long n, float soft, float g, int device, int rank, int world,
                        const void* unique_id)
{
    if (world < 1 || rank < 0 || rank >= world || (unsigned long)world > n) return MURBHIP_E_INVALID;
    if (world > MURB_SYM_MAX_RANKS) return MURBHIP_E_INVALID;
    if (world > 1 && !unique_id) return MURBHIP_E_INVALID;
    if ((world > 1 || unique_id) && !rccl().ok) return MURBHIP_E_NO_RCCL;
    RC_TRY(create_common(out, n, soft, g, world, 1, &device, &rank, 1, true));
    if (world > 1 || unique_id) {
        rccl_id_t id;
        std::memcpy(&id, unique_id, sizeof id);
        int rc = hip_rc(hipSetDevice(device));
        if (rc == 0) rc = nccl_rc(rccl().CommInitRank(&(*out)->shards[0].comm_rccl, world, id, rank));
        if (rc != 0) { murbhip_destroy(*out); *out = nullptr; return rc; }
    }
    return 0;
}

int murbhip_destroy(murbhip_ctx* c)
{
    if (!c) return 0;
    delete c->crew;
    c->crew = nullptr;
    for (Shard& sh : c->shards) {
        (void)hipSetDevice(sh.device);
        drain(sh.compute); drain(sh.comm); drain(sh.compute_low);
        if (sh.comm_rccl && rccl().ok) rccl().CommDestroy(sh.comm_rccl);
        for (hipEvent_t& e : sh.prof) release_event(e);
        for (hipEvent_t* e : {&sh.ev_tri, &sh.ev_integrated, &sh.ev_gathered, &sh.ev_rowsum, &sh.ev_reduced}) release_event(*e);
        for (hipStream_t* q : {&sh.compute_low, &sh.compute, &sh.comm}) release_stream(*q);
        release(sh.rec[0], sh.rec[1], sh.vel, sh.accp, sh.acc_out, sh.phi_out, sh.mass, sh.radius, sh.metrics);
        if (sh.metrics_host) (void)hipHostFree(sh.metrics_host);
        release(sh.herm_rec, sh.herm_vel, sh.herm_a0, sh.herm_j0, sh.herm_part, sh.herm_ctl);
        if (sh.herm_ctl_host) (void)hipHostFree(sh.herm_ctl_host);
        release(sh.blk_ctl, sh.blk_ticks, sh.blk_levels, sh.blk_list, sh.blk_rec, sh.blk_vel, sh.blk_part);
        release(sh.nn_idx, sh.nn_r2, sh.enc);
        release(sh.herm_phi, sh.pot_sums);
        release(sh.fld_in, sh.fld_pts, sh.fld_out, sh.fld_part);
        release(sh.trc_state, sh.trc_pts, sh.trc_part);
        release(sh.knn_part_r2, sh.knn_part_idx, sh.knn_list_r2, sh.knn_list_idx, sh.knn_rho, sh.knn_sums);
        if (sh.pot_sums_host) (void)hipHostFree(sh.pot_sums_host);
        if (sh.blk_ctl_host) (void)hipHostFree(sh.blk_ctl_host);
        release(sh.sym_items, sh.sym_send, sh.sym_recv, sh.sym_p2p, sh.sym_tri_acc, sh.sym_acc64);
        free_sym_set(sh, sh.sym_main); free_sym_set(sh, sh.sym_tri);
    }
    delete c;
    return 0;
}

int murbhip_upload(murbhip_ctx* c, const float* qx, const float* qy, const float* qz, const float* vx, const float* vy,
                   const float* vz, const float* m)
{
    if (!c || !qx || !qy || !qz || !vx || !vy || !vz || !m) return MURBHIP_E_INVALID;
    RC_TRY(murbhip_sync(c));
    {
        double reach2 = (double)c->soft2;
        for (const float* q : {qx, qy, qz}) {
            float lo = q[0], hi = q[0];
            bool finite = true;
            for (unsigned long i = 0; i < c->in.n; ++i) {
                lo = std::min(lo, q[i]);
                hi = std::max(hi, q[i]);
                finite = finite && std::isfinite(q[i]);
            }
            const double extent = finite ? (double)hi - (double)lo : (double)INFINITY;
            reach2 += extent * extent;
        }
        c->sym_wide_needed = sym_wide_needed(std::sqrt(reach2), std::sqrt((double)c->soft2));
    }
    std::vector<float4> rec(c->in.slots, make_float4(0.f, 0.f, 0.f, 0.f));
    for (int r = 0; r < c->in.world; ++r) {
        unsigned long first, count;
        partition(c->in.n, c->in.world, r, &first, &count);
        pack_records(qx, qy, qz, m, c->g, true, first, count, (unsigned long)r * c->in.slice, rec);
    }
    for (Shard& sh : c->shards) {
        HIP_TRY(hipSetDevice(sh.device));
        std::vector<float4> vel(c->in.slice, make_float4(0.f, 0.f, 0.f, 0.f));
        pack_records(vx, vy, vz, nullptr, 0.f, false, sh.first, sh.count, 0, vel);
        HIP_TRY(hipMemcpy(sh.rec[0], rec.data(), rec.size() * sizeof(float4), hipMemcpyHostToDevice));
        HIP_TRY(hipMemcpy(sh.rec[1], rec.data(), rec.size() * sizeof(float4), hipMemcpyHostToDevice));
        HIP_TRY(hipMemcpy(sh.vel, vel.data(), vel.size() * sizeof(float4), hipMemcpyHostToDevice));
        RC_TRY(shard_alloc(sh, sh.mass, c->in.slice * sizeof(float)));
        std::vector<float> mass(c->in.slice, 0.f);
        std::copy(m + sh.first, m + sh.first + sh.count, mass.begin());
        HIP_TRY(hipMemcpy(sh.mass, mass.data(), mass.size() * sizeof(float), hipMemcpyHostToDevice));
    }
    bodies_loaded(c);
    if (c->contact) RC_TRY(enqueue_radii_lanes(c));
    return 0;
}

namespace {
MurbRandBase rand_base_words(unsigned int seed)
{
    int32_t st[MURB_RAND_DEG];
    int32_t word = seed == 0 ? 1 : (int32_t)seed;
    st[0] = word;
    for (int i = 1; i < MURB_RAND_DEG; ++i) {
        const long hi = word / 127773, lo = word % 127773;
        word = (int32_t)(16807 * lo - 2836 * hi);
        if (word < 0) word += 2147483647;
        st[i] = word;
    }
    const int discard = 10 * MURB_RAND_DEG, first = discard - MURB_RAND_DEG, count = 2 * MURB_RAND_DEG - 1;
    MurbRandBase b{};
    int f = 3, r = 0;
// ... 774 lines not shown

int murbhip_step(murbhip_ctx* c, float dt)
{
    return murbhip_steps(c, dt, 1);
}

int murbhip_steps(murbhip_ctx* c, float dt, int iterations)
{
    if (!c || iterations < 0) return MURBHIP_E_INVALID;
    if (!c->uploaded || c->blk_open) return MURBHIP_E_STATE;
    for (int i = 0; i < iterations; ++i) {
        if (c->integrator == 2) { RC_TRY(enqueue_hermite(c, dt, 1)); continue; }
        RC_TRY(enqueue_iteration(c, dt, 1));
        if (c->integrator == 1) { c->lf_half = true; c->lf_last_dt = dt; }
    }
    return 0;
}

int murbhip_integrate_host_acc(murbhip_ctx* c, const float* ax, const float* ay, const float* az, float dt)
{
    if (!c || !ax || !ay || !az) return MURBHIP_E_INVALID;
    if (!c->uploaded || c->lf_half) return MURBHIP_E_STATE;
    std::vector<float4> part(c->in.slice);
    for (Shard& sh : c->shards) {
        HIP_TRY(hipSetDevice(sh.device));
        if (c->gather_pending) HIP_TRY(hipStreamWaitEvent(sh.compute, sh.ev_gathered, 0));
        std::fill(part.begin(), part.end(), make_float4(0.f, 0.f, 0.f, 0.f));
        for (unsigned long k = 0; k < sh.count; ++k)
            part[k] = make_float4(ax[sh.first + k], ay[sh.first + k], az[sh.first + k], 0.f);
        RC_TRY(ensure_accp(c, sh));
        HIP_TRY(hipMemcpyAsync(sh.accp, part.data(), part.size() * sizeof(float4), hipMemcpyHostToDevice, sh.compute));
        HIP_TRY(hipStreamSynchronize(sh.compute));
        RC_TRY(enqueue_integrate(c, sh, 1, dt, 1, nullptr, 0));
    }
    if (c->in.world > 1) {
        RC_TRY(crew_run(c, [&](Shard& sh) { return shard_exchange(c, sh, c->cur ^ 1, 0); }));
        c->gather_pending = true;
    }
    c->cur ^= 1;
    invalidate_cached_forces(c);
    return 0;
}

namespace {
int ensure_acc_for_readout(murbhip_ctx* c)
{
    if (c->lf_half && !c->acc_current) RC_TRY(enqueue_iteration(c, 0.f, 0));
    return 0;
}

int device_metrics(murbhip_ctx* c, bool want_phi, double (&sums)[MURB_METRIC_VALUES], double* pair_sum = nullptr,
                   bool phi_has_self = true)
{
    if (!pair_sum && c->metrics_serial == c->state_serial && (c->metrics_with_phi || !want_phi)) {
        RC_TRY(murbhip_sync(c));
        for (int k = 0; k < MURB_METRIC_VALUES; ++k) sums[k] = c->metrics_sums[k];
        return 0;
    }
    const MetricsLayout l = metrics_layout(c);
    for (Shard& sh : c->shards) {
        HIP_TRY(hipSetDevice(sh.device));
        RC_TRY(shard_alloc(sh, sh.metrics, l.total * sizeof(double)));
        if (c->gather_pending) HIP_TRY(hipStreamWaitEvent(sh.compute, sh.ev_gathered, 0));
        MurbMetricsArgs a{};
        a.rec = sh.rec[c->cur];
        a.vel = sh.vel;
        a.mass = sh.mass;
        a.phi = want_phi ? sh.phi_out : nullptr;
        a.acc = sh.acc_out;
        a.out = sh.metrics;
        a.i_first_slot = (int)((unsigned long)sh.rank * c->in.slice);
        a.count = (int)sh.count;
        a.acc_stride = (unsigned int)c->in.slice;
        a.half_dt = c->lf_half ? 0.5f * c->lf_last_dt : 0.f;
        a.g_over_soft = phi_has_self ? (double)c->g / std::sqrt((double)c->soft2) : 0.0;
        hipLaunchKernelGGL(murb_metrics_kernel, dim3((unsigned)l.blocks), dim3(256), 0, sh.compute, a);
        RC_TRY(hip_rc(hipGetLastError()));
        if (!sh.metrics_host) HIP_TRY(hipHostMalloc((void**)&sh.metrics_host, l.total * sizeof(double), hipHostMallocDefault));
        HIP_TRY(hipMemcpyAsync(sh.metrics_host, sh.metrics, (pair_sum ? l.total : l.pe_main) * sizeof(double), hipMemcpyDeviceToHost, sh.compute));
    }
    RC_TRY(murbhip_sync(c));
    for (double& v : sums) v = 0.0;
    if (pair_sum) *pair_sum = 0.0;
    for (Shard& sh : c->shards) {
        const double* const host = sh.metrics_host;
        for (size_t b = 0; b < l.blocks; ++b)
            for (int k = 0; k < MURB_METRIC_VALUES; ++k) sums[k] += host[b * MURB_METRIC_VALUES + k];
        if (!pair_sum) continue;
        if (sh.sym_main.part) for (int k = 0; k < kPeSumBlocks; ++k) *pair_sum += host[l.pe_main + k];
        if (sh.sym_tri.part) for (int k = 0; k < kPeSumBlocks; ++k) *pair_sum += host[l.pe_tri + k];
        for (size_t b = 0; b < l.own_blocks * MURB_PE_DIAG_SPLIT; ++b) *pair_sum += host[l.pe_diag + b];
    }
    for (int k = 0; k < MURB_METRIC_VALUES; ++k) c->metrics_sums[k] = sums[k];
    c->metrics_serial = c->state_serial;
    c->metrics_with_phi = want_phi;
    return 0;
}
}

int murbhip_energy(murbhip_ctx* c, double* kinetic, double* potential)
{
    if (!c || !kinetic || !potential) return MURBHIP_E_INVALID;
    if (!c->uploaded || c->blk_open) return MURBHIP_E_STATE;
    const Plan main_plan = current_plan(c);
    if (main_plan.symmetric && !c->energy_sweep) {
        const MetricsLayout l = metrics_layout(c);
        for (Shard& sh : c->shards) {
            if (sh.metrics) continue;
            HIP_TRY(hipSetDevice(sh.device));
            RC_TRY(shard_alloc(sh, sh.metrics, l.total * sizeof(double)));
        }
        if (!(c->acc_current && c->pe_current)) {
            c->acc_current = false;
            c->want_pe = true;
            const int rc = enqueue_iteration(c, 0.f, 0);
            c->want_pe = false;
            RC_TRY(rc);
        }
        for (Shard& sh : c->shards) {
            HIP_TRY(hipSetDevice(sh.device));
            const size_t at[2] = {l.pe_main, l.pe_tri};
            int k = 0;
            for (SymSet* st : {&sh.sym_main, &sh.sym_tri}) {
                const size_t off = at[k++];
                if (!st->part || st->passes.size() > 1) continue;
                hipLaunchKernelGGL(murb_sym_pe_sum_kernel, dim3(kPeSumBlocks), dim3(1024), 0, sh.compute, st->part + 3 * st->comp_stride,
                                   (unsigned long)(st->comp_stride / MURB_SYM_R + 1), sh.metrics + off, 0);
                RC_TRY(hip_rc(hipGetLastError()));
            }
            hipLaunchKernelGGL(murb_sym_pe_diag_kernel, dim3((unsigned)(l.own_blocks * MURB_PE_DIAG_SPLIT)), dim3(256), 0, sh.compute, sh.rec[c->cur],
                               (int)(sh.rank * l.own_blocks), c->soft2, sh.metrics + l.pe_diag);
            RC_TRY(hip_rc(hipGetLastError()));
        }
        double sums[MURB_METRIC_VALUES], pair_sum = 0.0;
        RC_TRY(device_metrics(c, false, sums, &pair_sum));
        *kinetic = sums[0];
        *potential = -pair_sum / (double)c->g;
        return 0;
    }
    RC_TRY(ensure_acc_for_readout(c));
    Plan p{};
    p.variant = kPotentialKernel;
    {
        const unsigned long tiles_local = c->in.slice / MURB_TILE_BODIES, tiles_remote = (c->in.slots - c->in.slice) / MURB_TILE_BODIES;
        p.parts_local = std::max(1, auto_parts(c->in, 1, c->in.slice, tiles_local));
        p.parts_remote = c->in.world > 1 ? std::max(1, std::min<int>(auto_parts(c->in, 1, c->in.slice, tiles_remote), kMaxParts / 2)) : 0;
    }
    const bool symmetric_sweep = main_plan.symmetric && c->in.world == 1 && !c->force_exchange;
    const bool symmetric_multi = main_plan.symmetric && !symmetric_sweep;
    for (Shard& sh : c->shards) {
        HIP_TRY(hipSetDevice(sh.device));
        RC_TRY(shard_alloc(sh, sh.phi_out, 3 * c->in.slice * sizeof(float)));
    }
    RC_TRY(drain_for_rebuild(c, main_plan));
    if (symmetric_multi) {
        RC_TRY(crew_run(c, [&](Shard& sh) { return shard_potential_sym_multi(c, sh, main_plan); }));
        c->reduce_pending = true;
    }
    for (Shard& sh : c->shards) {
        if (symmetric_multi) break;
        HIP_TRY(hipSetDevice(sh.device));
        if (c->gather_pending) HIP_TRY(hipStreamWaitEvent(sh.compute, sh.ev_gathered, 0));
        if (symmetric_sweep) {
            RC_TRY(build_sym_schedule(c, sh, main_plan));
            if (sh.sym_main.passes.size() > 1) {
                RC_TRY(enqueue_sym_passes(c, sh, true));
                MurbIntegrateArgs a{};
                a.rec_in = sh.rec[c->cur]; a.rec_out = sh.rec[c->cur ^ 1]; a.vel = sh.vel;
                a.acc_out = sh.phi_out;
                a.acc64 = sh.sym_acc64; a.acc64_stride = (unsigned int)c->in.slots;
                a.count = (int)sh.count; a.acc_stride = (unsigned int)c->in.slice;
                hipLaunchKernelGGL(murb_integrate_kernel, dim3((unsigned)((c->in.slice / 2 + 255) / 256)), dim3(256), 0, sh.compute, a);
                RC_TRY(hip_rc(hipGetLastError()));
                continue;
            }
            RC_TRY(enqueue_sym_launch(c, sh, 0, sh.sym_items_total, false, nullptr, true));
            RC_TRY(enqueue_sym_rowsum(sh.sym_main, sh.phi_out, (unsigned int)c->in.slots, sh.compute));
            continue;
        }
        RC_TRY(enqueue_force(c, sh, p, 0));
        if (c->in.world > 1) RC_TRY(enqueue_force(c, sh, p, 1));
        RC_TRY(enqueue_integrate(c, sh, p.parts_local + p.parts_remote, 0.f, 0, nullptr, -1, sh.phi_out));
    }
    double sums[MURB_METRIC_VALUES];
    RC_TRY(device_metrics(c, true, sums, nullptr, main_plan.symmetric));
    *kinetic = sums[0];
    *potential = sums[1];
    return 0;
}

int murbhip_moments(murbhip_ctx* c, double* out10)
{
    if (!c || !out10) return MURBHIP_E_INVALID;
    if (!c->uploaded || c->blk_open) return MURBHIP_E_STATE;
    RC_TRY(ensure_acc_for_readout(c));
    double sums[MURB_METRIC_VALUES];
    RC_TRY(device_metrics(c, false, sums));
    std::memcpy(out10, sums + 2, 10 * sizeof(double));
    return 0;
}

int murbhip_set_option(murbhip_ctx* c, const char* key, long value)
{
    if (!c || !key) return MURBHIP_E_INVALID;
    const std::string k(key);
    if (k == "solo_shard" || k == "force_exchange") c->acc_current = false;
    const auto plan_key = [c](auto& field, auto v) {
        if (field != v) { c->acc_current = false; c->pe_current = false; c->metrics_serial = c->state_serial - 1; }
        field = v;
    };
    if (k == "variant") { if (value < 0 || value > kNumVariants) return MURBHIP_E_INVALID; plan_key(c->in.variant, (int)value); }
    else if (k == "jsplit") { if (value < 0 || value > kMaxParts / 2) return MURBHIP_E_INVALID; plan_key(c->in.jsplit, (int)value); }
    else if (k == "xcd_order") plan_key(c->xcd_order, value ? 1 : 0);
    else if (k == "pad_aware") plan_key(c->pad_aware, value ? 1 : 0);
    else if (k == "energy_sweep") c->energy_sweep = value ? 1 : 0;
    else if (k == "sym_wide") {
        if (value < -1 || value > 1) return MURBHIP_E_INVALID;
        plan_key(c->sym_wide, (int)value);
    }
    else if (k == "fuse_integrate") plan_key(c->in.fuse_integrate, value ? 1 : 0);
    else if (k == "exchange_p2p") {
        if (value && (c->exchange != 1 || !rccl().Send || !rccl().Recv)) return MURBHIP_E_STATE;
        RC_TRY(murbhip_sync(c));
        c->exchange_p2p = value ? 1 : 0;
    }
    else if (k == "tri_div") { if (value != 0 && value != 1 && value != 2 && value != 4 && value != 8) return MURBHIP_E_INVALID; plan_key(c->in.tri_div, (int)value); }
    else if (k == "init_libm_fma") { if (value < -1 || value > 1) return MURBHIP_E_INVALID; c->init_libm_fma = (int)value; }
    else if (k == "tri_first_pct") { if (value < 0 || value > 100) return MURBHIP_E_INVALID; plan_key(c->tri_first_pct, (int)value); }
    else if (k == "taper") { if (value < -1 || value > 100) return MURBHIP_E_INVALID; plan_key(c->in.taper, (int)value); }
    else if (k == "sym_pass_mb") { if (value < 0) return MURBHIP_E_INVALID; plan_key(c->in.sym_pass_mb, value); }
    else if (k == "diag_tri") { if (value < -1 || value > 1) return MURBHIP_E_INVALID; plan_key(c->in.diag_tri, (int)value); }
    else if (k == "sym_red") { if (value < -1 || value > 1) return MURBHIP_E_INVALID; plan_key(c->in.sym_red, (int)value); }
    else if (k == "sym_waves") { if (value != 0 && value != 4 && value != 8) return MURBHIP_E_INVALID; plan_key(c->in.sym_waves, (int)value); }
    else if (k == "overlap") { if (value < 0 || value > 2) return MURBHIP_E_INVALID; plan_key(c->overlap, (int)value); }
    else if (k == "integrator") {
        if (value < 0 || value > 2) return MURBHIP_E_INVALID;
        if (c->lf_half && value != c->integrator) return MURBHIP_E_STATE;
        if (value == 2 && (c->in.world != 1 || c->shards.size() != 1 || c->force_exchange)) return MURBHIP_E_STATE;
        if (value != 2 && (c->nearest || c->contact || c->potential)) return MURBHIP_E_STATE;
        if (value != 2 && c->tracers) return MURBHIP_E_STATE;
        c->integrator = (int)value;
    }
    else if (k == "evolve_batch") {
        if (value < 0 || value > kEvolveBatch) return MURBHIP_E_INVALID;
        c->evolve_batch = (int)value;
    }
    else if (k == "nearest" || k == "contact" || k == "potential") RC_TRY(set_side_option(c, k, value));
    else if (k == "block_units") {
        if (value < 0 || value > kBlockMaxUnits) return MURBHIP_E_INVALID;
        c->block_units = (int)value;
    }
    else if (k == "solo_shard") c->solo_shard = (int)value;
    else if (k == "cu_reserve") {
        if (value < 0 || value > c->in.cu_count / 2) return MURBHIP_E_INVALID;
        if ((int)value != c->cu_reserve) {
            RC_TRY(murbhip_sync(c));
            for (Shard& sh : c->shards) {
                HIP_TRY(hipSetDevice(sh.device));
                HIP_TRY(hipStreamDestroy(sh.compute)); sh.compute = nullptr;
                HIP_TRY(hipStreamDestroy(sh.compute_low)); sh.compute_low = nullptr;
                RC_TRY(create_compute_streams(c, sh, (int)value));
            }
            c->cu_reserve = (int)value;
        }
    }
    else if (k == "force_exchange") {
        if (value && c->exchange == 1 && !c->shards[0].comm_rccl) return MURBHIP_E_STATE;
        if (value && c->integrator == 2) return MURBHIP_E_STATE;
        c->force_exchange = value ? 1 : 0;
    }
    else if (k == "profile") {
        if (value < 0 || value > 2) return MURBHIP_E_INVALID;
        RC_TRY(murbhip_sync(c));
        c->profile = (int)value;
        for (Shard& sh : c->shards) {
            HIP_TRY(hipSetDevice(sh.device));
            if (c->profile && sh.prof.empty()) {
                sh.prof.resize(2 * kProfPairs);
                sh.prof_kind.assign(kProfPairs, 0);
                for (hipEvent_t& e : sh.prof) HIP_TRY(hipEventCreate(&e));
            }
            sh.prof_used = 0;
            sh.sym_launches = 0;
        }
    } else return MURBHIP_E_INVALID;
    return 0;
}

int murbhip_get_info(murbhip_ctx* c, const char* key, double* value)
{
    if (!c || !key || !value) return MURBHIP_E_INVALID;
    const std::string k(key);
    const Plan p = current_plan(c);
    if (k == "cu_count") *value = c->in.cu_count;
    else if (k == "clock_mhz") *value = c->clock_mhz;
    else if (k == "n") *value = (double)c->in.n;
    else if (k == "slots") *value = (double)c->in.slots;
    else if (k == "world") *value = c->in.world;
    else if (k == "cu_reserve") *value = c->cu_reserve;
    else if (k == "sym_passes") *value = c->shards[0].sym_main.passes.empty() ? 0.0 : (double)c->shards[0].sym_main.passes.size();
    else if (k == "rank") *value = c->shards[0].rank;
    else if (k == "jsplit") *value = p.symmetric ? (double)p.split
                                     : p.persistent ? (double)p.sched[0].nblocks / std::max(resident_blocks(c->in), 1)
                                                    : (double)(p.parts_local + p.parts_remote);
    else if (k == "hermite_parts") *value = hermite_parts(c->in);
    else if (k == "block_units") *value = block_units(c);
    else if (k == "block_grid") *value = block_grid(c);
    else if (k == "nearest") *value = c->nearest;
    else if (k == "encounter_count") *value = c->contact ? 0.0 : (double)c->enc_count;
    else if (k == "contact") *value = c->contact;
    else if (k == "potential") *value = c->potential;
    else if (k == "contact_count") *value = c->contact ? (double)c->enc_count : 0.0;
    else if (k == "block_steps") *value = c->blk_info[0];
    else if (k == "block_body_steps") *value = c->blk_info[1];
    else if (k == "block_clamped") *value = c->blk_info[2];
    else if (k == "block_max_active") *value = c->blk_info[3];
    else if (k == "sym_waves") *value = p.symmetric ? p.waves : 0;
    else if (k == "sym_wide") *value = p.symmetric && sym_wide_chosen(c->sym_wide, c->sym_wide_needed) ? 1 : 0;
    else if (k == "taper") *value = p.symmetric ? p.taper : 0;
    else if (k == "workgroups") *value = p.persistent ? p.sched[0].nblocks + (c->in.world > 1 ? p.sched[1].nblocks : 0) : 0;
    else if (k == "variant") *value = p.variant;
    else if (k == "interactions_per_launch") *value = c->interactions_per_launch;
    else if (k == "device_bytes") { double b = 0; for (Shard& sh : c->shards) b += (double)sh.bytes; *value = b; }
    else if (k == "sym_launches") { double v = 0; for (Shard& sh : c->shards) v += (double)sh.sym_launches; *value = v; }
    else if (k == "spans_dropped") {
        *value = 0;
        for (Shard& sh : c->shards) if (!sh.prof.empty() && sh.prof_used + 2 > sh.prof.size()) *value = 1;
    }
    else if (k == "force_launches" || k == "force_ms_avg" || k == "force_ms_total" || k.rfind("span_", 0) == 0 || k == "compute_wait_ms_per_step") {
        static const char* const names[kProfKinds] = {"force", "tri1", "rect", "tri2", "reduce_scatter", "all_gather", "wait_gather",
                                                      "wait_reduce", "step", "field", "tidal", "tracer", "knn"};
        RC_TRY(murbhip_sync(c));
        double total[kProfKinds] = {0};
        size_t count[kProfKinds] = {0};
        for (Shard& sh : c->shards) {
            HIP_TRY(hipSetDevice(sh.device));
            for (size_t i = 0; i + 1 < sh.prof_used; i += 2) {
                float ms = 0.f;
                HIP_TRY(hipEventElapsedTime(&ms, sh.prof[i], sh.prof[i + 1]));
                const int kind = sh.prof_kind[i / 2];
                total[kind] += ms; ++count[kind];
            }
        }
        const double f_total = total[kProfForce] + total[kProfTri1] + total[kProfRect] + total[kProfTri2];
        const size_t f_count = count[kProfForce] + count[kProfTri1] + count[kProfRect] + count[kProfTri2];
        if (k == "force_launches") *value = (double)f_count;
        else if (k == "force_ms_total") *value = f_total;
        else if (k == "force_ms_avg") *value = f_count ? f_total / (double)f_count : 0.0;
        else if (k == "compute_wait_ms_per_step")
            *value = count[kProfStep] ? (total[kProfWaitGather] + total[kProfWaitReduce]) / (double)count[kProfStep] : 0.0;
        else {
            const bool avg = k.size() > 7 && k.compare(k.size() - 7, 7, "_ms_avg") == 0;
            const bool cnt = k.size() > 6 && k.compare(k.size() - 6, 6, "_count") == 0;
            if (!avg && !cnt) return MURBHIP_E_INVALID;
            const std::string name = k.substr(5, k.size() - 5 - (avg ? 7 : 6));
            int kind = -1;
            for (int q = 0; q < kProfKinds; ++q) if (name == names[q]) kind = q;
            if (kind < 0) return MURBHIP_E_INVALID;
            *value = avg ? (count[kind] ? total[kind] / (double)count[kind] : 0.0) : (double)count[kind];
        }
    } else return MURBHIP_E_INVALID;
    return 0;
}

}
```

### nbody-eurohpc_amd/murbhip/__init__.py

```python
import ctypes as C
import os

import numpy as np

_HERE = os.path.dirname(os.path.abspath(__file__))
LIB_PATH = os.environ.get("MURBHIP_LIBRARY") or os.path.join(_HERE, "..", "lib", "libmurbhip.so")
G = np.float32(6.67384e-11)

_fp = C.POINTER(C.c_float)


class MurbHipError(RuntimeError):
    def __init__(self, code, what):
        self.code = code
        super().__init__(f"{what}: {error_string(code)} (code {code})")


_lib = None


def lib():
    global _lib
    if _lib is None:
        path = os.path.normpath(LIB_PATH)
        if not os.path.exists(path):
            raise FileNotFoundError(f"{path} is missing: build it with `make -C nbody-eurohpc_amd` "
                                    "(there is no CPU fallback for the HIP path)")
        L = C.CDLL(path)
        L.murbhip_version.restype = C.c_int
        L.murbhip_error_string.restype = C.c_char_p
        L.murbhip_error_string.argtypes = [C.c_int]
        L.murbhip_partition.argtypes = [C.c_ulong, C.c_int, C.c_int, C.POINTER(C.c_ulong), C.POINTER(C.c_ulong)]
        L.murbhip_slice_slots.restype = C.c_ulong
        L.murbhip_slice_slots.argtypes = [C.c_ulong, C.c_int]
        L.murbhip_slot_of_body.restype = C.c_ulong
        L.murbhip_slot_of_body.argtypes = [C.c_ulong, C.c_int, C.c_ulong]
        L.murbhip_schedule_items.argtypes = [C.c_ulong, C.c_int, C.c_int, C.c_int, C.POINTER(C.c_int), C.c_ulong,
                                             C.POINTER(C.c_ulong), C.POINTER(C.c_ulong)]
        L.murbhip_schedule_layout.argtypes = [C.c_ulong] + [C.c_int] * 7 + [C.POINTER(C.c_long), C.c_ulong, C.POINTER(C.c_ulong),
                                                                            C.POINTER(C.c_long), C.c_ulong, C.POINTER(C.c_ulong),
                                                                            C.POINTER(C.c_ulong), C.POINTER(C.c_ulong)]
        L.murbhip_device_count.argtypes = [C.POINTER(C.c_int)]
        L.murbhip_create.argtypes = [C.POINTER(C.c_void_p), C.c_ulong, C.c_float, C.c_float, C.c_int]
        L.murbhip_create_sharded.argtypes = [C.POINTER(C.c_void_p), C.c_ulong, C.c_float, C.c_float, C.c_int,
                                             C.POINTER(C.c_int), C.c_int]
        L.murbhip_unique_id.argtypes = [C.c_void_p]
        L.murbhip_create_rank.argtypes = [C.POINTER(C.c_void_p), C.c_ulong, C.c_float, C.c_float, C.c_int, C.c_int,
                                          C.c_int, C.c_void_p]
        L.murbhip_destroy.argtypes = [C.c_void_p]
        L.murbhip_upload.argtypes = [C.c_void_p] + [_fp] * 7
        L.murbhip_init_bodies.argtypes = [C.c_void_p, C.c_char_p, C.c_ulong]
        L.murbhip_download_mass.argtypes = [C.c_void_p, _fp, _fp]
        L.murbhip_download_state.argtypes = [C.c_void_p] + [_fp] * 6
        L.murbhip_download_acc.argtypes = [C.c_void_p] + [_fp] * 3
        L.murbhip_compute_acc.argtypes = [C.c_void_p]
        L.murbhip_compute_acc_jerk.argtypes = [C.c_void_p]
        L.murbhip_download_jerk.argtypes = [C.c_void_p] + [_fp] * 3
        L.murbhip_evolve.argtypes = [C.c_void_p, C.c_double, C.c_double, C.c_double, C.c_float, C.c_float, C.c_ulong,
                                     C.POINTER(C.c_double)]
        L.murbhip_evolve_dts.argtypes = [C.c_void_p, _fp, C.c_ulong, C.POINTER(C.c_ulong)]
        L.murbhip_evolve_block.argtypes = [C.c_void_p, C.c_float, C.c_ulong, C.c_double, C.c_double, C.c_int, C.c_ulong,
                                           C.POINTER(C.c_double)]
        L.murbhip_block_state.argtypes = [C.c_void_p, C.POINTER(C.c_uint), C.POINTER(C.c_int)]
        L.murbhip_block_set_levels.argtypes = [C.c_void_p, C.POINTER(C.c_int), C.c_int]
        L.murbhip_download_nearest.argtypes = [C.c_void_p, C.POINTER(C.c_int), _fp]
        L.murbhip_set_encounter.argtypes = [C.c_void_p, C.c_float]
        L.murbhip_encounters.argtypes = [C.c_void_p, C.POINTER(C.c_int), C.POINTER(C.c_int), _fp, C.c_ulong, C.POINTER(C.c_ulong),
                                         C.POINTER(C.c_double)]
        L.murbhip_upload_radii.argtypes = [C.c_void_p, _fp]
        L.murbhip_download_contact.argtypes = [C.c_void_p, C.POINTER(C.c_int), _fp]
        L.murbhip_contacts.argtypes = [C.c_void_p, C.POINTER(C.c_int), C.POINTER(C.c_int), _fp, C.c_ulong, C.POINTER(C.c_ulong),
                                       C.POINTER(C.c_double)]
        L.murbhip_download_potential.argtypes = [C.c_void_p, _fp]
        L.murbhip_potential_energy.argtypes = [C.c_void_p, C.POINTER(C.c_double)]
        L.murbfield_at.argtypes = [C.c_void_p, C.c_ulong] + [_fp] * 6 + [C.POINTER(C.c_int)] + [_fp] * 7
        L.murbfield_of.argtypes = [C.c_void_p, C.c_ulong, C.POINTER(C.c_int)] + [_fp] * 7
        L.murbfield_layout.argtypes = [C.c_ulong, C.c_long, C.c_long, C.POINTER(C.c_ulong)]
        L.murbfield_set_option.argtypes = [C.c_void_p, C.c_char_p, C.c_long]
        L.murbfield_get_option.argtypes = [C.c_void_p, C.c_char_p, C.POINTER(C.c_long)]
        L.murbtidal_at.argtypes = [C.c_void_p, C.c_ulong] + [_fp] * 3 + [C.POINTER(C.c_int)] + [_fp] * 6
        L.murbtidal_of.argtypes = [C.c_void_p, C.c_ulong, C.POINTER(C.c_int)] + [_fp] * 6
        _ip = C.POINTER(C.c_int)
        L.murbknn_of.argtypes = [C.c_void_p, C.c_int, C.c_ulong, _ip, _ip, _fp]
        L.murbknn_at.argtypes = [C.c_void_p, C.c_int, C.c_ulong] + [_fp] * 3 + [_ip, _ip, _fp]
        L.murbdensity_of.argtypes = [C.c_void_p, C.c_int, C.c_ulong, _ip, _fp]
        L.murbdensity_centre.argtypes = [C.c_void_p, C.c_int, C.POINTER(C.c_double)]
        L.murbknn_merge.argtypes = [C.c_int, _ip, _fp, _ip, _fp, _ip, _fp]
        L.murbknn_density.argtypes = [C.c_int, _ip, _fp, _fp, C.c_float, _fp]
        L.murbtracer_upload.argtypes = [C.c_void_p, C.c_ulong] + [_fp] * 6
        L.murbtracer_download.argtypes = [C.c_void_p] + [_fp] * 6
        L.murbtracer_download_forces.argtypes = [C.c_void_p] + [_fp] * 6
        L.murbtracer_compute.argtypes = [C.c_void_p]
        L.murbtracer_count.argtypes = [C.c_void_p, C.POINTER(C.c_ulong)]
        L.murbtracer_clear.argtypes = [C.c_void_p]
        L.murbtracer_set_option.argtypes = [C.c_void_p, C.c_char_p, C.c_long]
        L.murbtracer_get_option.argtypes = [C.c_void_p, C.c_char_p, C.POINTER(C.c_long)]
        L.murbtracer_validate.argtypes = [C.c_ulong] + [_fp] * 6
        L.murbhip_warmup.argtypes = [C.c_void_p, C.c_double]
        L.murbhip_step.argtypes = [C.c_void_p, C.c_float]
        L.murbhip_steps.argtypes = [C.c_void_p, C.c_float, C.c_int]
        L.murbhip_integrate_host_acc.argtypes = [C.c_void_p] + [_fp] * 3 + [C.c_float]
        L.murbhip_sync.argtypes = [C.c_void_p]
        L.murbhip_energy.argtypes = [C.c_void_p, C.POINTER(C.c_double), C.POINTER(C.c_double)]
        L.murbhip_moments.argtypes = [C.c_void_p, C.POINTER(C.c_double)]
        L.murbhip_set_option.argtypes = [C.c_void_p, C.c_char_p, C.c_long]
        L.murbhip_get_info.argtypes = [C.c_void_p, C.c_char_p, C.POINTER(C.c_double)]
        _lib = L
    return _lib


EXPORTS = ("murbhip_version murbhip_error_string murbhip_partition murbhip_slice_slots murbhip_slot_of_body "
           "murbhip_schedule_items murbhip_schedule_layout "
           "murbhip_device_count murbhip_create murbhip_create_sharded murbhip_unique_id murbhip_create_rank "
           "murbhip_destroy murbhip_upload murbhip_init_bodies murbhip_download_mass murbhip_download_state murbhip_download_acc murbhip_compute_acc "
           "murbhip_compute_acc_jerk murbhip_download_jerk murbhip_evolve murbhip_evolve_dts "
           "murbhip_evolve_block murbhip_block_state murbhip_block_set_levels "
           "murbhip_download_nearest murbhip_set_encounter murbhip_encounters "
           "murbhip_upload_radii murbhip_download_contact murbhip_contacts "
           "murbhip_download_potential murbhip_potential_energy "
           "murbhip_warmup murbhip_step murbhip_steps murbhip_integrate_host_acc murbhip_sync murbhip_energy murbhip_moments murbhip_set_option "
           "murbhip_get_info").split()


FIELD_EXPORTS = "murbfield_at murbfield_of murbfield_layout murbfield_set_option murbfield_get_option".split()
FIELD_OPTIONS = ("field_chunks", "field_batch")
TIDAL_EXPORTS = "murbtidal_at murbtidal_of".split()
TIDAL_KEYS = ("txx", "tyy", "tzz", "txy", "txz", "tyz")
TRACER_EXPORTS = ("murbtracer_upload murbtracer_download murbtracer_download_forces murbtracer_compute murbtracer_count "
                  "murbtracer_clear murbtracer_set_option murbtracer_get_option murbtracer_validate").split()
TRACER_OPTIONS = ("tracer_chunks", "tracer_batch", "tracer_dt")
KNN_EXPORTS = "murbknn_of murbknn_at murbdensity_of murbdensity_centre murbknn_merge murbknn_density".split()
KNN_KMAX = 32
CENTRE_KEYS = ("x", "r_core", "rho_core", "rho_sum", "used", "left_out")


def error_string(code):
    return lib().murbhip_error_string(code).decode()


def _check(code, what):
    if code != 0:
        raise MurbHipError(code, what)


def _ptr(a):
    return a.ctypes.data_as(_fp)


def _f32(a):
    return np.ascontiguousarray(a, dtype=np.float32)


def partition(n, world, rank):
    first, count = C.c_ulong(), C.c_ulong()
    _check(lib().murbhip_partition(n, world, rank, C.byref(first), C.byref(count)), "murbhip_partition")
    return first.value, count.value


def slice_slots(n, world):
    return lib().murbhip_slice_slots(n, world)


def slot_of_body(n, world, i):
    return lib().murbhip_slot_of_body(n, world, i)


def schedule_items(n, world, rank, split=1):
    count, own = C.c_ulong(), C.c_ulong()
    _check(lib().murbhip_schedule_items(n, world, rank, split, None, 0, C.byref(count), C.byref(own)),
           "murbhip_schedule_items")
    items = np.zeros((count.value, 2), np.int32)
    _check(lib().murbhip_schedule_items(n, world, rank, split, items.ctypes.data_as(C.POINTER(C.c_int)), count.value,
                                        C.byref(count), C.byref(own)), "murbhip_schedule_items")
    return items, own.value


def schedule_layout(n, world, rank, split=1, waves=4, taper=0, tri_first_pct=50, exchange_mode=False, diag_tri=False, tri_div=1):
    ni, nr, fm, ft = C.c_ulong(), C.c_ulong(), C.c_ulong(), C.c_ulong()
    args = (n, world, rank, split, waves, taper + (256 if diag_tri else 0) + 512 * {1: 0, 2: 1, 4: 2, 8: 3}[tri_div], tri_first_pct,
            int(exchange_mode))
    _check(lib().murbhip_schedule_layout(*args, None, 0, C.byref(ni), None, 0, C.byref(nr), C.byref(fm), C.byref(ft)),
           "murbhip_schedule_layout")
    items = np.zeros((ni.value, 8), np.int64)
    rows = np.zeros((nr.value, 7), np.int64)
    lp = C.POINTER(C.c_long)
    _check(lib().murbhip_schedule_layout(*args, items.ctypes.data_as(lp), ni.value, C.byref(ni), rows.ctypes.data_as(lp), nr.value,
                                         C.byref(nr), C.byref(fm), C.byref(ft)), "murbhip_schedule_layout")
    return items, rows, fm.value, ft.value


def field_layout(n, chunks=0, batch=0, count=0):
    out = (C.c_ulong * 4)(0, 0, 0, count)
    _check(lib().murbfield_layout(n, chunks, batch, out), "murbfield_layout")
    tiles = (n + 511) // 512
    k = int(out[0])
    return {"chunks": k, "groups": int(out[1]), "batches": int(out[2]), "rows": int(out[3]), "tiles": tiles,
            "ranges": [(tiles * c // k, tiles * (c + 1) // k) for c in range(k)]}


def tidal_matrix(d):
    t = [np.asarray(d[k]) for k in TIDAL_KEYS]
    m = np.empty(t[0].shape + (3, 3), t[0].dtype)
    for (a, b), x in zip(((0, 0), (1, 1), (2, 2), (0, 1), (0, 2), (1, 2)), t):
        m[..., a, b] = m[..., b, a] = x
    return m


def knn_merge(idx_a, r2_a, idx_b, r2_b):
    ia, ib = (np.ascontiguousarray(x, np.int32) for x in (idx_a, idx_b))
    ra, rb = _f32(r2_a), _f32(r2_b)
    k = ia.shape[0]
    if any(x.shape != (k,) for x in (ia, ib, ra, rb)):
        raise ValueError("four lists of one length")
    io, ro = np.zeros(k, np.int32), np.zeros(k, np.float32)
    ip = C.POINTER(C.c_int)
    _check(lib().murbknn_merge(k, ia.ctypes.data_as(ip), _ptr(ra), ib.ctypes.data_as(ip), _ptr(rb), io.ctypes.data_as(ip), _ptr(ro)),
           "murbknn_merge")
    return io, ro


def knn_density(idx, r2, masses, soft):
    i, r, m = np.ascontiguousarray(idx, np.int32), _f32(r2), _f32(masses)
    if i.shape != r.shape or i.ndim != 1:
        raise ValueError("idx and r2 are one list")
    if i.size and i.max() >= m.shape[0]:
        raise ValueError("an index has no mass")
    out = np.zeros(1, np.float32)
    _check(lib().murbknn_density(i.shape[0], i.ctypes.data_as(C.POINTER(C.c_int)), _ptr(r), _ptr(m), float(np.float32(soft)), _ptr(out)),
           "murbknn_density")
    return out[0]


def _centre_dict(out):
    return {"x": np.array(out[:3]), "r_core": out[3], "rho_core": out[4], "rho_sum": out[5], "used": int(out[6]), "left_out": int(out[7])}


def device_count():
    c = C.c_int(0)
    rc = lib().murbhip_device_count(C.byref(c))
    return c.value if rc == 0 else 0


def unique_id():
    buf = C.create_string_buffer(128)
    _check(lib().murbhip_unique_id(buf), "murbhip_unique_id")
    return buf.raw


class Simulation:

    def __init__(self, n, soft=2e8, g=G, device=0, devices=None, exchange="copy", rank=None, world=None, uid=None):
        self.n = int(n)
        self._h = C.c_void_p()
        L = lib()
        if devices is not None:
            arr = (C.c_int * len(devices))(*devices)
            _check(L.murbhip_create_sharded(C.byref(self._h), self.n, soft, g, len(devices), arr,
                                            {"copy": 0, "rccl": 1}[exchange]), "murbhip_create_sharded")
        elif rank is not None:
            _check(L.murbhip_create_rank(C.byref(self._h), self.n, soft, g, device, rank, world, uid),
                   "murbhip_create_rank")
        else:
            _check(L.murbhip_create(C.byref(self._h), self.n, soft, g, device), "murbhip_create")

    def upload(self, s):
        a = [_f32(s[k]) for k in ("qx", "qy", "qz", "vx", "vy", "vz", "m")]
        for x in a:
            if x.shape[0] < self.n:
                raise ValueError("state arrays shorter than n")
        _check(lib().murbhip_upload(self._h, *[_ptr(x) for x in a]), "murbhip_upload")

    def init_bodies(self, scheme="galaxy", seed=0):
        _check(lib().murbhip_init_bodies(self._h, scheme.encode(), seed), "murbhip_init_bodies")

    def masses(self, with_radii=False):
        m = np.zeros(self.n, np.float32)
        r = np.zeros(self.n, np.float32) if with_radii else None
        _check(lib().murbhip_download_mass(self._h, _ptr(m), _ptr(r) if with_radii else None), "murbhip_download_mass")
        return (m, r) if with_radii else m

    def state(self):
        out = {k: np.zeros(self.n, np.float32) for k in ("qx", "qy", "qz", "vx", "vy", "vz")}
        _check(lib().murbhip_download_state(self._h, *[_ptr(out[k]) for k in ("qx", "qy", "qz", "vx", "vy", "vz")]),
               "murbhip_download_state")
        return out

    def acc(self):
        a = [np.zeros(self.n, np.float32) for _ in range(3)]
        _check(lib().murbhip_download_acc(self._h, *[_ptr(x) for x in a]), "murbhip_download_acc")
        return tuple(a)

    def compute_acc(self):
        _check(lib().murbhip_compute_acc(self._h), "murbhip_compute_acc")

    def compute_acc_jerk(self):
        _check(lib().murbhip_compute_acc_jerk(self._h), "murbhip_compute_acc_jerk")

    def jerk(self):
        j = [np.zeros(self.n, np.float32) for _ in range(3)]
        _check(lib().murbhip_download_jerk(self._h, *[_ptr(x) for x in j]), "murbhip_download_jerk")
        return tuple(j)

    def warmup(self, milliseconds=50.0):
        _check(lib().murbhip_warmup(self._h, milliseconds), "murbhip_warmup")

    def step(self, dt=3600.0):
        _check(lib().murbhip_step(self._h, dt), "murbhip_step")

    def steps(self, dt, iterations):
        _check(lib().murbhip_steps(self._h, dt, iterations), "murbhip_steps")

    def evolve(self, duration, eta=0.02, eta_start=0.01, dt_min=0.0, dt_max=None, max_steps=1_000_000):
        out = (C.c_double * 5)()
        _check(lib().murbhip_evolve(self._h, duration, eta, eta_start, dt_min, duration if dt_max is None else dt_max,
                                    max_steps, out), "murbhip_evolve")
        return {"time": out[0], "steps": int(out[1]), "dt_min": out[2], "dt_max": out[3], "dt_next": out[4]}

    def evolve_dts(self):
        count = C.c_ulong()
        _check(lib().murbhip_evolve_dts(self._h, None, 0, C.byref(count)), "murbhip_evolve_dts")
        dts = np.zeros(count.value, np.float32)
        if count.value:
            _check(lib().murbhip_evolve_dts(self._h, _ptr(dts), count.value, C.byref(count)), "murbhip_evolve_dts")
        return dts

    def evolve_block(self, dt_max, blocks=1, eta=0.02, eta_start=0.01, kmax=12, max_steps=2 ** 62):
        out = (C.c_double * 8)()
        _check(lib().murbhip_evolve_block(self._h, dt_max, blocks, eta, eta_start, kmax, max_steps, out), "murbhip_evolve_block")
        return {"time": out[0], "steps": int(out[1]), "body_steps": int(out[2]), "dt_min": out[3], "dt_max": out[4],
                "clamped": int(out[5]), "max_active": int(out[6]), "synchronised": bool(out[7])}

    def block_state(self):
        ticks, levels = np.zeros(self.n, np.uint32), np.zeros(self.n, np.int32)
        _check(lib().murbhip_block_state(self._h, ticks.ctypes.data_as(C.POINTER(C.c_uint)), levels.ctypes.data_as(C.POINTER(C.c_int))),
               "murbhip_block_state")
        return ticks, levels

    def set_block_levels(self, levels, kmax):
        lv = np.ascontiguousarray(levels, np.int32)
        if lv.shape[0] < self.n:
            raise ValueError("levels shorter than n")
# ... 533 lines not shown
```

Baseline: 6698 billion interactions/s.

## Pair two j blocks per symmetric work item to reuse i-row registers

Adds a paired-j mode to the symmetric force kernel: each work item loads two j blocks into shared memory and walks both against the same i registers, doubling the j accumulators and reducing each block separately. This is meant to cut per-item overhead and i-side reloads and partial-sum writes. It also adds prefetch of the next j tile with scheduling barriers. It is enabled by default for single-GPU runs with N >= 200000, 4 waves and force-only form. The cost is higher register and LDS pressure, which may reduce occupancy.

After: 6748 billion interactions/s (median of 6 runs). No clear change (+0.7%).

```diff
diff --git a/include/murbplan.h b/include/murbplan.h
--- /dev/null
+++ b/include/murbplan.h
@@ -0,0 +1,17 @@
+#ifndef MURBPLAN_H_
+#define MURBPLAN_H_
+
+#ifdef __cplusplus
+extern "C" {
+#endif
+
+int murbplan_layout_jpair(unsigned long n, int split, int waves, int taper_pct, long* items, unsigned long item_capacity,
+                          unsigned long* item_count, long* rows, unsigned long row_capacity, unsigned long* row_count,
+                          unsigned long* floats_main);
+
+int murbplan_jpair_chosen(int option, unsigned long n, int world, int exchange_mode, int waves, int red, int energy_form);
+
+#ifdef __cplusplus
+}
+#endif
+#endif
diff --git a/nbody-eurohpc_amd/csrc/murb_choose.h b/nbody-eurohpc_amd/csrc/murb_choose.h
--- a/nbody-eurohpc_amd/csrc/murb_choose.h
+++ b/nbody-eurohpc_amd/csrc/murb_choose.h
@@ -22,6 +22,7 @@
     int taper = -1;
     int diag_tri = -1;
     int sym_red = -1;
+    int sym_jpair = -1;
     int fuse_integrate = 1;
     long sym_pass_mb = 0;
     int tri_div = 0;
@@ -46,6 +47,7 @@
     int taper;
     bool diag_tri;
     int red;
+    bool jpair;
     MurbSchedule sched[2];
 };
 
@@ -53,6 +55,13 @@
 constexpr double kSymFastMinSoft = 0x1p-40;
 inline bool sym_wide_needed(double reach, double soft) { return !(reach <= kSymFastMaxReach && soft >= kSymFastMinSoft); }
 inline bool sym_wide_chosen(int option, bool needed) { return option < 0 ? needed : option != 0; }
+
+constexpr unsigned long kSymJpairMinBodies = 200000;
+inline bool sym_jpair_chosen(int option, unsigned long n, int world, bool exchange_mode, int waves, int red, bool energy_form)
+{
+    if (world != 1 || exchange_mode || energy_form || waves != 4 || red != 1) return false;
+    return option < 0 ? n >= kSymJpairMinBodies : option > 0;
+}
 
 inline int resident_blocks(const PlanInputs& in) { return std::max(in.resident_per_cu, 1) * std::max(in.cu_count, 1); }
 
@@ -145,6 +154,7 @@
         p.taper = in.taper >= 0 ? in.taper : (in.world > 1 ? 0 : (small ? sp.taper : (in.n <= 600000 ? 5 : 0)));
         p.diag_tri = in.diag_tri >= 0 ? in.diag_tri != 0 : (small && sp.diag_tri);
         p.red = in.sym_red >= 0 ? in.sym_red : 1;
+        p.jpair = sym_jpair_chosen(in.sym_jpair, in.n, in.world, false, p.waves, p.red, false);
         p.persistent = false;
         p.parts_local = p.parts_remote = 0;
         return p;
@@ -191,7 +201,7 @@
 }
 
 inline SymLayoutKey sym_layout_key(const PlanInputs& in, const Plan& p, bool exchange_mode, int overlap, int tri_first_pct, bool xcd_order,
-                                   bool pad_aware)
+                                   bool pad_aware, bool energy_form = false)
 {
     SymLayoutKey k;
     k.split = p.split; k.waves = p.waves; k.taper = p.taper; k.diag_tri = p.diag_tri;
@@ -202,6 +212,7 @@
     k.budget_floats = sym_pass_budget(in) / (3 * sizeof(float));
     k.tri_div = plan_tri_div(in, p);
     k.pad_aware = pad_aware;
+    k.jpair = p.jpair && sym_jpair_chosen(in.sym_jpair, in.n, in.world, exchange_mode, p.waves, p.red, energy_form);
     return k;
 }
 
diff --git a/nbody-eurohpc_amd/csrc/murb_ctx.h b/nbody-eurohpc_amd/csrc/murb_ctx.h
--- a/nbody-eurohpc_amd/csrc/murb_ctx.h
+++ b/nbody-eurohpc_amd/csrc/murb_ctx.h
@@ -63,6 +63,7 @@
     MurbSymItem* sym_items = nullptr;
     int sym_items_own = 0, sym_items_total = 0;
     SymLayoutKey key;
+    bool sym_paired = false;
     int sym_red = 0;
     int sym_t1 = 0;
     SymSet sym_main;
@@ -211,6 +212,7 @@
     unsigned long metrics_serial = 0;
     bool metrics_with_phi = false;
     double metrics_sums[MURB_METRIC_VALUES] = {0};
+    bool phi_sweep = false;
     bool want_pe = false;
     bool pe_current = false;
     float lf_last_dt = 0.f;
diff --git a/nbody-eurohpc_amd/csrc/murb_kernels_sym.h b/nbody-eurohpc_amd/csrc/murb_kernels_sym.h
--- a/nbody-eurohpc_amd/csrc/murb_kernels_sym.h
+++ b/nbody-eurohpc_amd/csrc/murb_kernels_sym.h
@@ -6,6 +6,12 @@
 
 #ifndef MURB_SYM_STEP_BARRIER
 #define MURB_SYM_STEP_BARRIER 1
+#endif
+#ifndef MURB_SYM2_BARRIER
+#define MURB_SYM2_BARRIER 2
+#endif
+#ifndef MURB_SYM2_PREFETCH
+#define MURB_SYM2_PREFETCH 1
 #endif
 
 struct MurbSymArgs {
@@ -148,14 +154,16 @@
     phi_j = __builtin_elementwise_fma(inv, (murb_f2)(gi), phi_j);
 }
 
-template <int WAVES, int ILOAD, int PHI, int RED, int DYN, int WIDE>
+template <int WAVES, int ILOAD, int PHI, int RED, int DYN, int WIDE, int JB = 1, int NB = JB>
 __device__ __forceinline__ void murb_sym_walk(const MurbSymArgs& a, const float4* tileA, const float4* tileB, float* stage,
                                               const int lane, const int wave, const int groups_per_wave,
                                               const unsigned int i_block_slot, const unsigned long out_off, const int out_stride,
                                               const float pe_scale, const int p_first,
-                                              const int p_sym, murb_f2 (&ajx)[MURB_SYM_STEPS], murb_f2 (&ajy)[MURB_SYM_STEPS],
-                                              murb_f2 (&ajz)[MURB_SYM_STEPS])
-{
+                                              const int p_sym, murb_f2 (&ajx)[MURB_SYM_STEPS * JB], murb_f2 (&ajy)[MURB_SYM_STEPS * JB],
+                                              murb_f2 (&ajz)[MURB_SYM_STEPS * JB])
+{
+    static_assert(NB >= 1 && NB <= JB, "a walk covers the item's first NB j blocks");
+    static_assert(JB == 1 || (JB == 2 && PHI == 0), "two j blocks per item: the force form only");
     constexpr int R = MURB_SYM_R;
     constexpr int NV = PHI == 2 ? 13 : 12;
     const float soft2 = a.soft2;
@@ -219,6 +227,30 @@
         for (int r = 0; r < R; ++r) { aix[r] = (murb_f2)(0.f); aiy[r] = (murb_f2)(0.f); aiz[r] = (murb_f2)(0.f); }
         murb_f2 pe = (murb_f2)(0.f);
 
+        if constexpr (JB == 2) {
+            float4 A = tileA[lane], B = tileB[lane];
+            {
+#pragma unroll
+                for (int p = 0; p < MURB_SYM_STEPS * NB; ++p) {
+                    const int pn = p + 1 < MURB_SYM_STEPS * NB ? p + 1 : p;
+                    float4 An, Bn;
+                    if (MURB_SYM2_PREFETCH) { An = tileA[pn * 64 + lane]; Bn = tileB[pn * 64 + lane]; }
+                    else { A = tileA[p * 64 + lane]; B = tileB[p * 64 + lane]; An = A; Bn = B; }
+                    if (DYN == 0 || p >= p_first) {
+                        const murb_f2 xj = {A.x, A.y}, yj = {A.z, A.w}, zj = {B.x, B.y}, gj = {B.z, B.w};
+                        const unsigned both = DYN ? murb_ones_if_ge(p, p_sym) : ~0u;
+#pragma unroll
+                        for (int r = 0; r < R; ++r) {
+                            const float gie = DYN ? murb_masked(gi[r], both) : gi[r];
+                            murb_interact_sym<WIDE>(xj, yj, zj, gj, xi[r], yi[r], zi[r], gie, soft2, aix[r], aiy[r], aiz[r], ajx[p], ajy[p],
+                                                    ajz[p]);
+                        }
+                    }
+                    if (MURB_SYM2_BARRIER && (p + 1) % (MURB_SYM2_BARRIER ? MURB_SYM2_BARRIER : 1) == 0) __builtin_amdgcn_sched_barrier(0);
+                    A = An; B = Bn;
+                }
+            }
+        } else
 #pragma unroll
         for (int p = 0; p < MURB_SYM_STEPS; ++p) {
             if (DYN == 0 || p >= p_first) {
@@ -260,12 +292,12 @@
     }
 }
 
-template <int MINW, int WAVES = 4, int ILOAD = 0, int PHI = 0, int RED = 0, int WIDE = 0>
+template <int MINW, int WAVES = 4, int ILOAD = 0, int PHI = 0, int RED = 0, int WIDE = 0, int JB = 1>
 __global__ __launch_bounds__(64 * WAVES, MINW) void murb_force_sym_kernel(const MurbSymArgs a)
 {
     constexpr int THREADS = 64 * WAVES;
-    __shared__ float4 tileA[MURB_SYM_PAIRS];
-    __shared__ float4 tileB[MURB_SYM_PAIRS];
+    __shared__ float4 tileA[MURB_SYM_PAIRS * JB];
+    __shared__ float4 tileB[MURB_SYM_PAIRS * JB];
     __shared__ murb_f2 scratch[WAVES / 2][3][MURB_SYM_PAIRS];
 
     const int lane = threadIdx.x & 63;
@@ -279,6 +311,7 @@
     const bool no_j_side = (flags & 1) != 0;
     const bool triangular = (flags & 2) != 0;
     const int p_first = (flags >> 8) & 15, p_sym = (flags >> 12) & 15;
+    const bool two = JB == 2 && (flags & MURB_SYM_ITEM_PAIRED) != 0;
 #ifdef MURB_LAB_BEGIN
     MURB_LAB_BEGIN();
 #endif
@@ -293,11 +326,24 @@
             else tileB[tile * MURB_TILE_PAIRS + in - MURB_TILE_PAIRS] = v;
         }
     }
+    if constexpr (JB == 2) {
+        if (two) {
+            const int J2 = __builtin_amdgcn_readfirstlane(it.J2);
+            const float4* src = a.rec + (unsigned long)J2 * (MURB_SYM_BLOCK / MURB_TILE_BODIES) * MURB_TILE_F4;
+#pragma unroll
+            for (int k = threadIdx.x; k < 2 * MURB_TILE_F4; k += THREADS) {
+                const int tile = k / MURB_TILE_F4, in = k % MURB_TILE_F4;
+                const float4 v = src[k];
+                if (in < MURB_TILE_PAIRS) tileA[MURB_SYM_PAIRS + tile * MURB_TILE_PAIRS + in] = v;
+                else tileB[MURB_SYM_PAIRS + tile * MURB_TILE_PAIRS + in - MURB_TILE_PAIRS] = v;
+            }
+        }
+    }
     __syncthreads();
 
-    murb_f2 ajx[MURB_SYM_STEPS], ajy[MURB_SYM_STEPS], ajz[MURB_SYM_STEPS];
-#pragma unroll
-    for (int p = 0; p < MURB_SYM_STEPS; ++p) { ajx[p] = (murb_f2)(0.f); ajy[p] = (murb_f2)(0.f); ajz[p] = (murb_f2)(0.f); }
+    murb_f2 ajx[MURB_SYM_STEPS * JB], ajy[MURB_SYM_STEPS * JB], ajz[MURB_SYM_STEPS * JB];
+#pragma unroll
+    for (int p = 0; p < MURB_SYM_STEPS * JB; ++p) { ajx[p] = (murb_f2)(0.f); ajy[p] = (murb_f2)(0.f); ajz[p] = (murb_f2)(0.f); }
 
     unsigned long out_off;
     int out_stride = MURB_SYM_R;
@@ -314,45 +360,57 @@
     }
     float* const stage = reinterpret_cast<float*>(&scratch[0][0][0]) + wave * ((PHI == 2 ? 13 : 12) * 80);
     if (triangular)
-        murb_sym_walk<WAVES, ILOAD, PHI, RED, 1, WIDE>(a, tileA, tileB, stage, lane, wave, groups_per_wave, (unsigned int)i_item_slot, out_off,
+        murb_sym_walk<WAVES, ILOAD, PHI, RED, 1, WIDE, JB, 1>(a, tileA, tileB, stage, lane, wave, groups_per_wave, (unsigned int)i_item_slot, out_off,
                                                  out_stride, 0.f, p_first, p_sym, ajx, ajy, ajz);
+    else if (JB == 1 || !two)
+        murb_sym_walk<WAVES, ILOAD, PHI, RED, 0, WIDE, JB, 1>(a, tileA, tileB, stage, lane, wave, groups_per_wave, (unsigned int)i_item_slot, out_off,
+                                                 out_stride, (i_item_slot / MURB_SYM_BLOCK == J) ? 0.f : 1.f, 0, 0, ajx, ajy, ajz);
     else
-        murb_sym_walk<WAVES, ILOAD, PHI, RED, 0, WIDE>(a, tileA, tileB, stage, lane, wave, groups_per_wave, (unsigned int)i_item_slot, out_off,
-                                                 out_stride, (i_item_slot / MURB_SYM_BLOCK == J) ? 0.f : 1.f, 0, 0, ajx, ajy, ajz);
+        murb_sym_walk<WAVES, ILOAD, PHI, RED, 0, WIDE, JB, JB>(a, tileA, tileB, stage, lane, wave, groups_per_wave, (unsigned int)i_item_slot, out_off,
+                                                 out_stride, 1.f, 0, 0, ajx, ajy, ajz);
 
     if (!no_j_side) {
         if constexpr (RED != 0) __syncthreads();
 #pragma unroll
-        for (int half = WAVES / 2; half >= 1; half >>= 1) {
-            if (wave >= half && wave < 2 * half) {
-#pragma unroll
-                for (int p = 0; p < MURB_SYM_STEPS; ++p) {
-                    scratch[wave - half][0][p * 64 + lane] = ajx[p];
-                    scratch[wave - half][1][p * 64 + lane] = ajy[p];
-                    scratch[wave - half][2][p * 64 + lane] = ajz[p];
+        for (int b = 0; b < JB; ++b) {
+            if (b == 1) {
+                if (!two) break;
+                __syncthreads();
+            }
+            constexpr int S = MURB_SYM_STEPS;
+#pragma unroll
+            for (int half = WAVES / 2; half >= 1; half >>= 1) {
+                if (wave >= half && wave < 2 * half) {
+#pragma unroll
+                    for (int p = 0; p < S; ++p) {
+                        scratch[wave - half][0][p * 64 + lane] = ajx[b * S + p];
+                        scratch[wave - half][1][p * 64 + lane] = ajy[b * S + p];
+                        scratch[wave - half][2][p * 64 + lane] = ajz[b * S + p];
+                    }
                 }
-            }
-            __syncthreads();
-            if (wave < half) {
-#pragma unroll
-                for (int p = 0; p < MURB_SYM_STEPS; ++p) {
-                    ajx[p] += scratch[wave][0][p * 64 + lane];
-                    ajy[p] += scratch[wave][1][p * 64 + lane];
-                    ajz[p] += scratch[wave][2][p * 64 + lane];
+                __syncthreads();
+                if (wave < half) {
+#pragma unroll
+                    for (int p = 0; p < S; ++p) {
+                        ajx[b * S + p] += scratch[wave][0][p * 64 + lane];
+                        ajy[b * S + p] += scratch[wave][1][p * 64 + lane];
+                        ajz[b * S + p] += scratch[wave][2][p * 64 + lane];
+                    }
                 }
-            }
-            if (half > 1) __syncthreads();
-        }
-        if (wave == 0) {
-            murb_f2* px = reinterpret_cast<murb_f2*>(a.part + it.joff);
-            murb_f2* py = reinterpret_cast<murb_f2*>(a.part + a.comp_stride + it.joff);
-            murb_f2* pz = reinterpret_cast<murb_f2*>(a.part + 2ul * a.comp_stride + it.joff);
-#pragma unroll
-            for (int p = 0; p < MURB_SYM_STEPS; ++p) {
-                px[p * 64 + lane] = ajx[p];
-                if constexpr (PHI != 1) {
-                    py[p * 64 + lane] = ajy[p];
-                    pz[p * 64 + lane] = ajz[p];
+                if (half > 1) __syncthreads();
+            }
+            if (wave == 0) {
+                const unsigned long joff = b == 0 ? it.joff : it.joff2;
+                murb_f2* px = reinterpret_cast<murb_f2*>(a.part + joff);
+                murb_f2* py = reinterpret_cast<murb_f2*>(a.part + a.comp_stride + joff);
+                murb_f2* pz = reinterpret_cast<murb_f2*>(a.part + 2ul * a.comp_stride + joff);
+#pragma unroll
+                for (int p = 0; p < S; ++p) {
+                    px[p * 64 + lane] = ajx[b * S + p];
+                    if constexpr (PHI != 1) {
+                        py[p * 64 + lane] = ajy[b * S + p];
+                        pz[p * 64 + lane] = ajz[b * S + p];
+                    }
                 }
             }
         }
diff --git a/nbody-eurohpc_amd/csrc/murb_plan.h b/nbody-eurohpc_amd/csrc/murb_plan.h
--- a/nbody-eurohpc_amd/csrc/murb_plan.h
+++ b/nbody-eurohpc_amd/csrc/murb_plan.h
@@ -43,11 +43,15 @@
                       std::vector<MurbSymBlockRows>& table, OutOf out_of)
 {
     std::map<int, int> index;
-    for (size_t k = first; k < end; ++k) { index[pieces[k].i_slot0 / MURB_SYM_BLOCK] = 0; if (pieces[k].j_side()) index[pieces[k].J] = 0; }
+    for (size_t k = first; k < end; ++k) {
+        index[pieces[k].i_slot0 / MURB_SYM_BLOCK] = 0;
+        if (pieces[k].j_side()) index[pieces[k].J] = 0;
+        if (pieces[k].paired()) index[pieces[k].J2] = 0;
+    }
     table.assign(index.size(), MurbSymBlockRows{});
     { int e = 0; for (auto& kv : index) { kv.second = e; const auto o = out_of(kv.first); table[e].out_slice = o.first; table[e].out_block = o.second; ++e; } }
     std::vector<std::map<int, int>> irow(index.size());
-    std::vector<int> item_irow(end - first), item_jrow(end - first);
+    std::vector<int> item_irow(end - first), item_jrow(end - first), item_jrow2(end - first, -1);
     for (size_t k = first; k < end; ++k) {
         const SymPiece& pc = pieces[k];
         const int bi = index[pc.i_slot0 / MURB_SYM_BLOCK];
@@ -55,6 +59,7 @@
         if (f == irow[bi].end()) f = irow[bi].emplace(pc.J, table[bi].ni++).first;
         item_irow[k - first] = f->second;
         item_jrow[k - first] = pc.j_side() ? table[index[pc.J]].nj++ : -1;
+        if (pc.paired()) item_jrow2[k - first] = table[index[pc.J2]].nj++;
     }
     size_t floats = 0;
     for (MurbSymBlockRows& br : table) {
@@ -71,6 +76,8 @@
         const MurbSymBlockRows& bi = table[index[pc.i_slot0 / MURB_SYM_BLOCK]];
         it.ioff = bi.base_i + (size_t)item_irow[k - first] * MURB_SYM_BLOCK + (size_t)(pc.i_slot0 % MURB_SYM_BLOCK);
         it.joff = pc.j_side() ? table[index[pc.J]].base_j + (size_t)item_jrow[k - first] * MURB_SYM_BLOCK : 0;
+        it.J2 = pc.J2;
+        it.joff2 = pc.paired() ? table[index[pc.J2]].base_j + (size_t)item_jrow2[k - first] * MURB_SYM_BLOCK : 0;
     }
     return floats;
 }
@@ -81,6 +88,7 @@
     std::vector<MurbSymBlockRows> table_main, table_tri;
     size_t floats_main = 0, floats_tri = 0;
     std::vector<SymPass> passes;
+    bool paired = false;
 };
 
 struct SymLayoutKey {
@@ -92,11 +100,12 @@
     size_t budget_floats = 0;
     int tri_div = 1;
     bool pad_aware = true;
+    bool jpair = false;
     bool operator==(const SymLayoutKey& o) const
     {
         return split == o.split && waves == o.waves && taper == o.taper && diag_tri == o.diag_tri && exchange_mode == o.exchange_mode &&
                overlap == o.overlap && tri_first_pct == o.tri_first_pct && xcd_order == o.xcd_order && budget_floats == o.budget_floats &&
-               tri_div == o.tri_div && pad_aware == o.pad_aware;
+               tri_div == o.tri_div && pad_aware == o.pad_aware && jpair == o.jpair;
     }
 };
 
@@ -125,6 +134,8 @@
     };
     build_pieces(key.xcd_order);
     if (!key.exchange_mode && key.xcd_order && cut_passes(pieces, key.budget_floats).size() > 1) build_pieces(false);
+    const bool jpair = key.jpair && W == 1 && !key.exchange_mode && key.waves == 4 && cut_passes(pieces, key.budget_floats).size() == 1;
+    if (jpair) sym_pair_pieces(pieces, piece_ends, fill, 16 * key.waves);
     size_t own_pieces = pieces.size();
     if (key.exchange_mode && flat.size() / 2 > (size_t)own) own_pieces = piece_ends.size() >= 2 ? piece_ends[piece_ends.size() - 2] : 0;
     L.items.assign(pieces.size(), MurbSymItem{});
@@ -138,13 +149,16 @@
     } else {
         L.passes.clear();
         std::vector<MurbSymBlockRows> table;
-        for (const auto& range : cut_passes(pieces, key.budget_floats)) {
+        const auto ranges = jpair ? std::vector<std::pair<size_t, size_t>>(1, std::make_pair((size_t)0, pieces.size())) : cut_passes(pieces, key.budget_floats);
+        for (const auto& range : ranges) {
             const size_t floats = layout_sym_set(pieces, range.first, range.second, key.waves, L.items, table, [&](int b) { return std::make_pair(0, b); });
             L.passes.push_back(SymPass{(int)range.first, (int)(range.second - range.first), (int)L.table_main.size(), (int)table.size(), floats});
             L.table_main.insert(L.table_main.end(), table.begin(), table.end());
             L.floats_main = std::max(L.floats_main, floats);
         }
     }
+    L.paired = false;
+    for (const SymPiece& pc : pieces) L.paired = L.paired || pc.paired();
     L.own = (int)own_pieces;
     L.t1 = t1 > 0 ? (int)piece_ends[0] : 0;
 }
diff --git a/nbody-eurohpc_amd/csrc/murb_schedule.h b/nbody-eurohpc_amd/csrc/murb_schedule.h
--- a/nbody-eurohpc_amd/csrc/murb_schedule.h
+++ b/nbody-eurohpc_amd/csrc/murb_schedule.h
@@ -2,6 +2,7 @@
 #define MURB_SCHEDULE_H_
 
 #include <algorithm>
+#include <utility>
 #include <vector>
 
 #include "murb_layout.h"
@@ -128,8 +129,10 @@
 
 struct SymPiece {
     int i_slot0, len, J, flags;
+    int J2 = -1;
     bool diag() const { return i_slot0 / MURB_SLICE_ALIGN == J; }
     bool j_side() const { return (flags & 1) == 0; }
+    bool paired() const { return J2 >= 0; }
 };
 constexpr int kSymStepBodies = 128;
 
@@ -175,6 +178,43 @@
     }
 }
 
+inline void sym_pair_pieces(std::vector<SymPiece>& pieces, std::vector<size_t>& piece_launch_ends, const SymFill& fill, int min_len)
+{
+    const auto whole = [&](const SymPiece& pc) {
+        const int real = std::min(MURB_SLICE_ALIGN, (fill.of(pc.i_slot0 / MURB_SLICE_ALIGN) + min_len - 1) / min_len * min_len);
+        return pc.len == real && pc.i_slot0 % MURB_SLICE_ALIGN == 0 && pc.flags == 0 && !pc.diag() && !pc.paired();
+    };
+    std::vector<SymPiece> out;
+    std::vector<size_t> ends;
+    out.reserve(pieces.size());
+    size_t first = 0;
+    for (const size_t end : piece_launch_ends) {
+        std::vector<std::pair<std::pair<int, int>, size_t>> at;
+        for (size_t k = first; k < end; ++k)
+            if (whole(pieces[k])) at.push_back({{pieces[k].i_slot0 / MURB_SLICE_ALIGN, pieces[k].J}, k});
+        std::sort(at.begin(), at.end());
+        std::vector<char> gone(end - first, 0);
+        for (size_t k = first; k < end; ++k) {
+            if (gone[k - first]) continue;
+            SymPiece pc = pieces[k];
+            if (whole(pc)) {
+                const std::pair<int, int> want{pc.i_slot0 / MURB_SLICE_ALIGN, pc.J + 1};
+                const auto f = std::lower_bound(at.begin(), at.end(), std::make_pair(want, (size_t)0));
+                if (f != at.end() && f->first == want && f->second > k && !gone[f->second - first]) {
+                    gone[f->second - first] = 1;
+                    pc.J2 = pc.J + 1;
+                    pc.flags |= 4;
+                }
+            }
+            out.push_back(pc);
+        }
+        ends.push_back(out.size());
+        first = end;
+    }
+    pieces.swap(out);
+    piece_launch_ends.swap(ends);
+}
+
 }
 
 #endif
diff --git a/nbody-eurohpc_amd/csrc/murb_sym_types.h b/nbody-eurohpc_amd/csrc/murb_sym_types.h
--- a/nbody-eurohpc_amd/csrc/murb_sym_types.h
+++ b/nbody-eurohpc_amd/csrc/murb_sym_types.h
@@ -13,7 +13,11 @@
     int flags;
     unsigned long ioff;
     unsigned long joff;
+    unsigned long joff2;
+    int J2;
+    int pad_;
 };
+#define MURB_SYM_ITEM_PAIRED 4
 
 
 #define MURB_SYM_MAX_RANKS 64
diff --git a/nbody-eurohpc_amd/csrc/murbhip.hip b/nbody-eurohpc_amd/csrc/murbhip.hip
--- a/nbody-eurohpc_amd/csrc/murbhip.hip
+++ b/nbody-eurohpc_amd/csrc/murbhip.hip
@@ -16,6 +16,7 @@
 #include "../../include/murbtidal.h"
 #include "../../include/murbknn.h"
 #include "../../include/murbtracer.h"
+#include "../../include/murbplan.h"
 #include "murb_init.h"
 #include "murb_ctx.h"
 
@@ -313,7 +314,8 @@
 inline bool exchange_mode(const murbhip_ctx* c) { return c->in.world > 1 || c->force_exchange; }
 SymLayoutKey layout_key(const murbhip_ctx* c, const Plan& p)
 {
-    return sym_layout_key(c->in, p, exchange_mode(c), c->overlap, c->tri_first_pct, c->xcd_order != 0, c->pad_aware != 0);
+    return sym_layout_key(c->in, p, exchange_mode(c), c->overlap, c->tri_first_pct, c->xcd_order != 0, c->pad_aware != 0,
+                          c->want_pe || c->phi_sweep);
 }
 
 inline bool sym_schedule_stale(const Shard& sh, const SymLayoutKey& key) { return !sh.sym_items || !(sh.key == key); }
@@ -344,6 +346,7 @@
     sh.sym_main.passes = L.passes;
     if (L.passes.size() > 1) RC_TRY(shard_alloc(sh, sh.sym_acc64, 3 * c->in.slots * sizeof(double)));
     sh.sym_items_own = L.own;
+    sh.sym_paired = L.paired;
     sh.sym_items_total = (int)L.items.size();
     sh.sym_t1 = L.t1;
     RC_TRY(shard_alloc(sh, sh.sym_items, L.items.size() * sizeof(MurbSymItem)));
@@ -367,7 +370,10 @@
 void launch_sym_t(int form, int count, hipStream_t stream, const MurbSymArgs& sa)
 {
     const dim3 grid((unsigned)count), block(64 * WAVES);
-    if (form == 1) hipLaunchKernelGGL((murb_force_sym_kernel<4, WAVES, 1, 1>), grid, block, 0, stream, sa);
+    if (form == 4) {
+        if constexpr (WAVES == 4) hipLaunchKernelGGL((murb_force_sym_kernel<2, 4, 1, 0, 1, WIDE, 2>), grid, block, 0, stream, sa);
+    }
+    else if (form == 1) hipLaunchKernelGGL((murb_force_sym_kernel<4, WAVES, 1, 1>), grid, block, 0, stream, sa);
     else if (form == 2) hipLaunchKernelGGL((murb_force_sym_kernel<4, WAVES, 1, 2, 1, WIDE>), grid, block, 0, stream, sa);
     else if (form == 3) hipLaunchKernelGGL((murb_force_sym_kernel<4, WAVES, 1, 0, 1, WIDE>), grid, block, 0, stream, sa);
     else hipLaunchKernelGGL((murb_force_sym_kernel<4, WAVES, 1, 0, 0, WIDE>), grid, block, 0, stream, sa);
@@ -392,7 +398,8 @@
     int rc_span = 0;
     const int sp = timed ? span_begin(c, sh, kind, stream, &rc_span) : -1;
     RC_TRY(rc_span);
-    const int form = potential ? 1 : (with_pe ? 2 : (sh.sym_red == 1 ? 3 : 0));
+    if (sh.sym_paired && (potential || with_pe || sh.sym_red != 1 || sh.key.waves != 4)) return MURBHIP_E_STATE;
+    const int form = potential ? 1 : (with_pe ? 2 : (sh.sym_paired ? 4 : (sh.sym_red == 1 ? 3 : 0)));
     const bool wide = sym_wide_chosen(c->sym_wide, c->sym_wide_needed);
     if (sh.key.waves == 8) { if (wide) launch_sym_t<8, 1>(form, count, stream, sa); else launch_sym_t<8, 0>(form, count, stream, sa); }
     else { if (wide) launch_sym_t<4, 1>(form, count, stream, sa); else launch_sym_t<4, 0>(form, count, stream, sa); }
@@ -1544,10 +1551,11 @@
     return 0;
 }
 
-int murbhip_schedule_layout(unsigned long n, int world, int rank, int split, int waves, int taper_pct, int tri_first_pct,
-                            int exchange_mode, long* items, unsigned long item_capacity, unsigned long* item_count, long* rows,
-                            unsigned long row_capacity, unsigned long* row_count, unsigned long* floats_main,
-                            unsigned long* floats_tri)
+namespace {
+int schedule_layout(unsigned long n, int world, int rank, int split, int waves, int taper_pct, int tri_first_pct,
+                    int exchange_mode, bool jpair, long* items, unsigned long item_capacity, unsigned long* item_count, long* rows,
+                    unsigned long row_capacity, unsigned long* row_count, unsigned long* floats_main,
+                    unsigned long* floats_tri)
 {
     if (world < 1 || world > MURB_SYM_MAX_RANKS || rank < 0 || rank >= world || !item_count || !row_count) return MURBHIP_E_INVALID;
     if (split != 1 && split != 2 && split != 4 && split != 8 && split != 16) return MURBHIP_E_INVALID;
@@ -1559,6 +1567,7 @@
     key.split = split; key.waves = waves; key.taper = taper_pct & 0xff; key.diag_tri = (taper_pct & 0x100) != 0;
     key.exchange_mode = exchange_mode != 0 || world > 1;
     key.overlap = 1; key.tri_first_pct = tri_first_pct; key.tri_div = 1 << ((taper_pct >> 9) & 3);
+    key.jpair = jpair;
     plan_sym_layout(world, rank, sym_fill(n, world), key, L);
     *item_count = L.items.size();
     *row_count = L.table_main.size() + L.table_tri.size();
@@ -1569,7 +1578,8 @@
         const bool ex = key.exchange_mode;
         for (size_t k = 0; k < L.items.size(); ++k) {
             const MurbSymItem& it = L.items[k];
-            long* o = items + 8 * k;
+            long* o = items + (jpair ? 10 : 8) * k;
+            if (jpair) { o[8] = it.J2; o[9] = (long)it.joff2; }
             o[0] = it.i_slot0; o[1] = (long)it.ngroups * waves * MURB_SYM_R; o[2] = it.J; o[3] = it.flags;
             o[4] = (ex && (int)k < L.own) ? 1 : 0;
             o[5] = (long)it.ioff; o[6] = (long)it.joff;
@@ -1586,6 +1596,29 @@
             }
     }
     return 0;
+}
+}
+
+int murbhip_schedule_layout(unsigned long n, int world, int rank, int split, int waves, int taper_pct, int tri_first_pct,
+                            int exchange_mode, long* items, unsigned long item_capacity, unsigned long* item_count, long* rows,
+                            unsigned long row_capacity, unsigned long* row_count, unsigned long* floats_main,
+                            unsigned long* floats_tri)
+{
+    return schedule_layout(n, world, rank, split, waves, taper_pct, tri_first_pct, exchange_mode, false, items, item_capacity, item_count, rows,
+                           row_capacity, row_count, floats_main, floats_tri);
+}
+
+int murbplan_jpair_chosen(int option, unsigned long n, int world, int exchange_mode, int waves, int red, int energy_form)
+{
+    return sym_jpair_chosen(option, n, world, exchange_mode != 0, waves, red, energy_form != 0) ? 1 : 0;
+}
+
+int murbplan_layout_jpair(unsigned long n, int split, int waves, int taper_pct, long* items, unsigned long item_capacity,
+                                  unsigned long* item_count, long* rows, unsigned long row_capacity, unsigned long* row_count,
+                                  unsigned long* floats_main)
+{
+    return schedule_layout(n, 1, 0, split, waves, taper_pct, 50, 0, true, items, item_capacity, item_count, rows, row_capacity, row_count,
+                           floats_main, nullptr);
 }
 
 int murbhip_device_count(int* count)
@@ -2666,6 +2699,7 @@
         HIP_TRY(hipSetDevice(sh.device));
         RC_TRY(shard_alloc(sh, sh.phi_out, 3 * c->in.slice * sizeof(float)));
     }
+    struct PhiSweep { murbhip_ctx* c; explicit PhiSweep(murbhip_ctx* c_) : c(c_) { c->phi_sweep = true; } ~PhiSweep() { c->phi_sweep = false; } } phi_sweep(c);
     RC_TRY(drain_for_rebuild(c, main_plan));
     if (symmetric_multi) {
         RC_TRY(crew_run(c, [&](Shard& sh) { return shard_potential_sym_multi(c, sh, main_plan); }));
@@ -2744,6 +2778,7 @@
     else if (k == "taper") { if (value < -1 || value > 100) return MURBHIP_E_INVALID; plan_key(c->in.taper, (int)value); }
     else if (k == "sym_pass_mb") { if (value < 0) return MURBHIP_E_INVALID; plan_key(c->in.sym_pass_mb, value); }
     else if (k == "diag_tri") { if (value < -1 || value > 1) return MURBHIP_E_INVALID; plan_key(c->in.diag_tri, (int)value); }
+    else if (k == "sym_jpair") { if (value < -1 || value > 1) return MURBHIP_E_INVALID; plan_key(c->in.sym_jpair, (int)value); }
     else if (k == "sym_red") { if (value < -1 || value > 1) return MURBHIP_E_INVALID; plan_key(c->in.sym_red, (int)value); }
     else if (k == "sym_waves") { if (value != 0 && value != 4 && value != 8) return MURBHIP_E_INVALID; plan_key(c->in.sym_waves, (int)value); }
     else if (k == "overlap") { if (value < 0 || value > 2) return MURBHIP_E_INVALID; plan_key(c->overlap, (int)value); }
@@ -2832,6 +2867,11 @@
     else if (k == "sym_waves") *value = p.symmetric ? p.waves : 0;
     else if (k == "sym_wide") *value = p.symmetric && sym_wide_chosen(c->sym_wide, c->sym_wide_needed) ? 1 : 0;
     else if (k == "taper") *value = p.symmetric ? p.taper : 0;
+    else if (k == "sym_jpair") {
+        const SymLayoutKey key = layout_key(c, p);
+        const Shard& sh = c->shards[0];
+        *value = p.symmetric && key.jpair && (sym_schedule_stale(sh, key) || sh.sym_paired) ? 1 : 0;
+    }
     else if (k == "workgroups") *value = p.persistent ? p.sched[0].nblocks + (c->in.world > 1 ? p.sched[1].nblocks : 0) : 0;
     else if (k == "variant") *value = p.variant;
     else if (k == "interactions_per_launch") *value = c->interactions_per_launch;
diff --git a/nbody-eurohpc_amd/murbhip/__init__.py b/nbody-eurohpc_amd/murbhip/__init__.py
--- a/nbody-eurohpc_amd/murbhip/__init__.py
+++ b/nbody-eurohpc_amd/murbhip/__init__.py
@@ -40,6 +40,10 @@
         L.murbhip_schedule_layout.argtypes = [C.c_ulong] + [C.c_int] * 7 + [C.POINTER(C.c_long), C.c_ulong, C.POINTER(C.c_ulong),
                                                                             C.POINTER(C.c_long), C.c_ulong, C.POINTER(C.c_ulong),
                                                                             C.POINTER(C.c_ulong), C.POINTER(C.c_ulong)]
+        L.murbplan_layout_jpair.argtypes = [C.c_ulong] + [C.c_int] * 3 + [C.POINTER(C.c_long), C.c_ulong, C.POINTER(C.c_ulong),
+                                                                                  C.POINTER(C.c_long), C.c_ulong, C.POINTER(C.c_ulong),
+                                                                                  C.POINTER(C.c_ulong)]
+        L.murbplan_jpair_chosen.argtypes = [C.c_int, C.c_ulong] + [C.c_int] * 5
         L.murbhip_device_count.argtypes = [C.POINTER(C.c_int)]
         L.murbhip_create.argtypes = [C.POINTER(C.c_void_p), C.c_ulong, C.c_float, C.c_float, C.c_int]
         L.murbhip_create_sharded.argtypes = [C.POINTER(C.c_void_p), C.c_ulong, C.c_float, C.c_float, C.c_int,
@@ -124,6 +128,7 @@
 
 FIELD_EXPORTS = "murbfield_at murbfield_of murbfield_layout murbfield_set_option murbfield_get_option".split()
 FIELD_OPTIONS = ("field_chunks", "field_batch")
+PLAN_EXPORTS = "murbplan_layout_jpair murbplan_jpair_chosen".split()
 TIDAL_EXPORTS = "murbtidal_at murbtidal_of".split()
 TIDAL_KEYS = ("txx", "tyy", "tzz", "txy", "txz", "tyz")
 TRACER_EXPORTS = ("murbtracer_upload murbtracer_download murbtracer_download_forces murbtracer_compute murbtracer_count "
@@ -187,6 +192,18 @@
     _check(lib().murbhip_schedule_layout(*args, items.ctypes.data_as(lp), ni.value, C.byref(ni), rows.ctypes.data_as(lp), nr.value,
                                          C.byref(nr), C.byref(fm), C.byref(ft)), "murbhip_schedule_layout")
     return items, rows, fm.value, ft.value
+
+
+def schedule_layout_jpair(n, split=1, waves=4, taper=0, diag_tri=False):
+    ni, nr, fm = C.c_ulong(), C.c_ulong(), C.c_ulong()
+    args = (n, split, waves, taper + (256 if diag_tri else 0))
+    _check(lib().murbplan_layout_jpair(*args, None, 0, C.byref(ni), None, 0, C.byref(nr), C.byref(fm)), "murbplan_layout_jpair")
+    items = np.zeros((ni.value, 10), np.int64)
+    rows = np.zeros((nr.value, 7), np.int64)
+    lp = C.POINTER(C.c_long)
+    _check(lib().murbplan_layout_jpair(*args, items.ctypes.data_as(lp), ni.value, C.byref(ni), rows.ctypes.data_as(lp), nr.value,
+                                               C.byref(nr), C.byref(fm)), "murbplan_layout_jpair")
+    return items, rows, fm.value
 
 
 def field_layout(n, chunks=0, batch=0, count=0):
```
